# apelykh/deep-audio-mixer

Hardware: AMD Instinct MI355X
Metric: stem-spectrogram-frames/sec (train) (higher is better)
Workload: dtype f32; 1 GPU; C3: model_resnet (ResNet18, 8 stems) train step incl. STFT front-end, 8-stem 3 s @ 44.1 kHz stereo clips, n_fft 2048 hop 1024 -> 8x1025x130 per clip; batch_per_gpu=8, global_batch=8, parallelism=dp1, hip_graph=True, world_size=1, device_index=0, grad_buckets=1, allreduce_overlap=False

## Files before the change

### deep-audio-mixer_amd/_lib.py

```python
import ctypes
import os

import torch
import torch.utils.data

_HERE = os.path.dirname(os.path.abspath(__file__))
LIB_PATH = os.environ.get('DAM_LIB_PATH') or os.path.join(_HERE, 'libdam_hip.so')

EXPECTED_ABI = 26

_STATUS = {0: 'DAM_OK', -1: 'DAM_ERR_BAD_ARG', -2: 'DAM_ERR_UNSUPPORTED', -3: 'DAM_ERR_LAUNCH',
           -4: 'DAM_ERR_WORKSPACE'}

c_i, c_i64, c_f, c_p = ctypes.c_int, ctypes.c_int64, ctypes.c_float, ctypes.c_void_p
c_d = ctypes.c_double

SIGNATURES = {
    'dam_arch': (ctypes.c_char_p, []),
    'dam_abi_version': (c_i, []),
    'dam_host_dontfork_pinned': (c_i, [c_p, c_p]),
    'dam_step_mark_create': (c_i, [c_p]),
    'dam_step_mark_record': (c_i, [c_p, c_p]),
    'dam_step_mark_wait': (c_i, [c_p, c_p]),
    'dam_step_mark_synchronize': (c_i, [c_p]),
    'dam_step_mark_destroy': (c_i, [c_p]),
    'dam_stft_twiddle_count': (c_i64, [c_i]),
    'dam_stft_fill_twiddles_host': (c_i, [c_i, c_p]),
    'dam_stft_logmag_f32': (c_i, [c_p, c_i, c_i64, c_i64, c_i, c_i64, c_p, c_p, c_p, c_i, c_i, c_f, c_i, c_p, c_p]),
    'dam_stft_logmag_strided_f32': (c_i, [c_p, c_i, c_i64, c_i64, c_i64, c_i64, c_i64, c_i, c_i64, c_i64, c_p, c_p, c_p,
                                          c_i, c_i, c_f, c_i, c_p, c_p, c_i, c_p]),
    'dam_stft_complex_f32': (c_i, [c_p, c_i, c_i64, c_i64, c_i, c_i64, c_i64, c_i64, c_p, c_p, c_p, c_i, c_i, c_p, c_p]),
    'dam_stft_complex_strided_f32': (c_i, [c_p, c_i, c_i64, c_i64, c_i64, c_i64, c_i64, c_i64, c_i64, c_i, c_i64, c_i64,
                                           c_p, c_p, c_p, c_i, c_i, c_p, c_p]),
    'dam_istft_workspace_bytes': (c_i64, [c_i64, c_i64, c_i, c_i, c_i64]),
    'dam_istft_f32': (c_i, [c_p, c_p, c_i64, c_i64, c_i, c_i, c_i64, c_p, c_p, c_p, c_p, c_i64, c_p]),
    'dam_augment_gains_f32': (c_i, [ctypes.c_uint64, c_p, c_i64, c_i, c_i, c_f, c_f, c_p, c_p]),
    'dam_conv_packed_weight_count': (c_i64, [c_i, c_i, c_i, c_i]),
    'dam_conv_pack_weights_f32': (c_i, [c_p, c_i, c_i, c_i, c_i, c_i, c_p, c_p]),
    'dam_conv_pack_weights_multi_f32': (c_i, [c_p, c_i, c_i64, c_p]),
    'dam_conv2d_tapgrid_f32': (c_i, [c_p, c_i, c_i, c_i, c_i, c_i, c_p, c_i, c_i, c_p, c_p, c_p, c_i, c_i, c_p] +
                               [c_i] * 17 + [c_p, c_p, c_p, c_p, c_p, c_p, c_i64, c_p, c_p]),
    'dam_conv_batch_bytes': (c_i64, []),
    'dam_conv_batch_init': (c_i, [c_p]),
    'dam_conv_batch_flush': (c_i, [c_p, c_p]),
    'dam_conv_last_launch': (c_i, [c_p]),
    'dam_conv2d_wgrad_workspace_floats': (c_i64, [c_i, c_i, c_i, c_i]),
    'dam_conv2d_wgrad_f32': (c_i, [c_p, c_i, c_i, c_i, c_i, c_i, c_p, c_p, c_i, c_p] + [c_i] * 9 +
                             [c_p, c_i, c_p, c_i64, c_p, c_p]),
    'dam_wgrad_queue_bytes': (c_i64, []),
    'dam_wgrad_queue_init': (c_i, [c_p]),
    'dam_wgrad_queue_pending': (c_i, [c_p]),
    'dam_wgrad_queue_flush': (c_i, [c_p, c_p]),
    'dam_wgrad_queue_set_batching': (c_i, [c_p, c_i]),
    'dam_bn_workspace_floats': (c_i64, [c_i]),
    'dam_bn_stats_f32': (c_i, [c_p, c_i64, c_i, c_p, c_p, c_p, c_p, c_p, c_f, c_f, c_p, c_p, c_p, c_p, c_p, c_p]),
    'dam_bn_finalize_f32': (c_i, [c_p, c_i, c_i, c_p, c_p, c_p, c_p, c_p, c_f, c_f, c_p, c_p, c_p, c_p, c_p]),
    'dam_conv1x1_pair_f32': (c_i, [c_p, c_p, c_i, c_p, c_p, c_i, c_i, c_i, c_i, c_i, c_i, c_p, c_i, c_i, c_i, c_i, c_i, c_p]),
    'dam_dgrad_s2_3x3_f32': (c_i, [c_p, c_p, c_p, c_p, c_i, c_i, c_i, c_i, c_i, c_p, c_i, c_i, c_p, c_p, c_p, c_p]),
    'dam_conv_s2_pair_fwd_f32': (c_i, [c_p, c_p, c_p, c_i, c_i, c_i, c_i, c_i, c_p, c_p, c_p, c_p, c_p, c_p]),
    'dam_bn_finalize_pair_f32': (c_i, [c_p, c_p, c_i, c_i, c_p, c_p, c_p]),
    'dam_strip_diag_counters': (c_i, [c_p, c_i]),
    'dam_bn_stats_partial_f32': (c_i, [c_p, c_i64, c_i, c_p, c_p, c_p]),
    'dam_bn_finalize_apply_f32': (c_i, [c_p, c_i, c_i, c_p, c_p, c_i64, c_p, c_p, c_p, c_i, c_p, c_p, c_p]),
    'dam_bn_eval_affine_f32': (c_i, [c_i, c_p, c_p, c_p, c_p, c_f, c_p, c_p, c_p, c_p, c_p]),
    'dam_bn_apply_f32': (c_i, [c_p, c_i64, c_i, c_p, c_p, c_p, c_p, c_p, c_i, c_p, c_p, c_p]),
    'dam_bn_stats_pair_f32': (c_i, [c_p, c_p, c_i64, c_i, c_p, c_p, c_p, c_p]),
    'dam_bn_pair_workspace_floats': (c_i64, [c_i]),
    'dam_bn_backward_pair_f32': (c_i, [c_p, c_p, c_p, c_i64, c_i, c_i] + [c_p] * 16),
    'dam_bn_backward_f32': (c_i, [c_p, c_p, c_p, c_i64, c_i, c_p, c_p, c_p, c_i, c_p, c_p, c_p, c_p, c_p, c_p, c_p, c_i, c_p]),
    'dam_channel_sum_f32': (c_i, [c_p, c_i64, c_i, c_i, c_p, c_p, c_p]),
    'dam_dropout_tick': (c_i, [c_p, c_i64, c_p, c_p]),
    'dam_dropout_apply_f32': (c_i, [c_p, c_i64, c_f, ctypes.c_uint64, c_p, c_p, c_p]),
    'dam_heads_fwd_f32': (c_i, [c_p, c_i, c_i, c_i, c_i, c_p, c_p, c_p, c_p, c_p, c_p, c_p]),
    'dam_heads_bwd_workspace_floats': (c_i64, [c_i, c_i, c_i, c_i]),
    'dam_heads_bwd_f32': (c_i, [c_p, c_p, c_p, c_i, c_i, c_i, c_i, c_p, c_p, c_p, c_p, c_p, c_p, c_p, c_p, c_p]),
    'dam_masksum_fwd_f32': (c_i, [c_p, c_p, c_i, c_i, c_i64, c_p, c_p]),
    'dam_masksum_workspace_floats': (c_i64, [c_i, c_i]),
    'dam_masksum_bwd_f32': (c_i, [c_p, c_p, c_i, c_i, c_i64, c_p, c_p, c_p]),
    'dam_masksum_mse_f32': (c_i, [c_p, c_p, c_p, c_i, c_i, c_i64, c_p, c_p, c_p, c_p, c_p]),
    'dam_adam_l2_step_f32': (c_i, [c_p, c_p, c_p, c_p, c_i64, c_p, c_p, c_f, c_f, c_f, c_f, c_f, c_f, c_p, c_p]),
    'dam_digest64_u32': (c_i, [c_p, c_i64, c_i64, c_i, c_i, c_p, c_p]),
    'dam_gains_smooth': (c_i, [c_p, c_i, c_i, c_i, c_i, c_p, c_p, c_p, c_p]),
    'dam_gain_ramp_apply': (c_i, [c_p, c_i, c_p, c_i64, c_i64, c_i64, c_i, c_p, c_i, c_p]),
    'dam_mixdown_workspace_elems': (c_i64, [c_i64]),
    'dam_mixdown_peak_normalize': (c_i, [c_p, c_i, c_p, c_i, c_i64, c_i64, c_i, c_i, c_p, c_i, c_p, c_p]),
    'dam_nchw_to_nhwc16_f32': (c_i, [c_p, c_i, c_i, c_i64, c_p, c_p]),
    'dam_loudness_kweight_coeffs': (c_i, [c_d, c_p]),
    'dam_loudness_workspace_bytes': (c_i64, [c_i64, c_i]),
    'dam_loudness_block_energy': (c_i, [c_p, c_i, c_i64, c_i, c_i64, c_i64, c_p, c_p, c_p, c_i, c_d, c_p, c_p, c_p]),
    'dam_loudness_batch_workspace_bytes': (c_i64, [c_i, c_i64, c_i, c_i]),
    'dam_loudness_block_energy_batch': (c_i, [c_p, c_i, c_i, c_i64, c_i, c_i64, c_i64, c_i64, c_p, c_i, c_p, c_p, c_p, c_i,
                                              c_d, c_p, c_p, c_p]),
    'dam_loudness_gate': (c_i, [c_p, c_i, c_i, c_i, c_p, c_p]),
    'dam_loudness_target_gains': (c_i, [c_p, c_p, c_i, c_p, c_p]),
    'dam_pcm_tile_frames': (c_i64, [c_i]),
    'dam_pcm_max_blocks': (c_i, []),
    'dam_pcm_encode': (c_i, [c_p, c_i, c_i, c_i64, c_p, c_i, c_i, c_i, ctypes.c_uint64, c_p, c_p, c_p]),
    'dam_true_peak_taps_host': (c_i, [c_p]),
    'dam_true_peak_tile_samples': (c_i64, []),
    'dam_true_peak_max_blocks': (c_i, []),
    'dam_true_peak_workspace_bytes': (c_i64, [c_i, c_i64, c_i]),
    'dam_true_peak_batch': (c_i, [c_p, c_i, c_i, c_i64, c_i, c_i64, c_i64, c_i64, c_p, c_i, c_p, c_p, c_p, c_p]),
    'dam_peak_limit_gains': (c_i, [c_p, c_p, c_i, c_i, c_d, c_p]),
    'dam_limiter_tile_samples': (c_i64, []),
    'dam_limiter_max_lookahead': (c_i, []),
    'dam_limiter_max_hold': (c_i, []),
    'dam_limiter_workspace_bytes': (c_i64, [c_i, c_i64]),
    'dam_limiter_apply': (c_i, [c_p, c_i, c_i, c_i64, c_i, c_i64, c_i64, c_i64, c_p, c_d, c_i, c_i, c_p, c_i, c_p, c_p, c_p, c_p]),
    'dam_loudness_window_power': (c_i, [c_p, c_i, c_i, c_i, c_i, c_p, c_p, c_p]),
    'dam_loudness_curve_stats': (c_i, [c_p, c_i, c_i, c_p, c_p]),
    'dam_loudness_profile_error': (c_i, [c_p, c_p, c_i, c_i, c_i, c_p, c_p, c_p]),
    'dam_spectrum_frames_per_block': (c_i, []),
    'dam_spectrum_max_bands': (c_i, []),
    'dam_spectrum_workspace_bytes': (c_i64, [c_i, c_i64, c_i, c_i]),
    'dam_spectrum_band_power': (c_i, [c_p, c_i, c_i, c_i, c_i, c_i64, c_i64, c_i64, c_i64, c_i64, c_p, c_i, c_p, c_p, c_i, c_i,
                                      c_p, c_i, c_p, c_p, c_p]),
    'dam_spectrum_balance_error': (c_i, [c_p, c_p, c_i, c_i, c_p, c_p, c_p]),
    'dam_gainfit_tile_samples': (c_i64, []),
    'dam_gainfit_workspace_bytes': (c_i64, [c_i, c_i64, c_i]),
    'dam_gainfit_moments': (c_i, [c_p, c_i, c_i, c_i, c_i64, c_i64, c_i64, c_i64, c_p, c_i, c_i64, c_i64, c_i, c_p, c_p, c_p]),
    'dam_gainfit_solve': (c_i, [c_p, c_i, c_i, c_i, c_d, c_p, c_p, c_p, c_p]),
    'dam_gainfit_gain_error': (c_i, [c_p, c_p, c_i, c_i, c_i, c_i, c_p, c_p, c_p, c_p]),
}
# ... 59 lines not shown
```

### deep-audio-mixer_amd/csrc/dam_conv.hip

```cpp
#include <cstdlib>
#include "dam_common.h"
#include "dam_conv_geo.h"
#include "dam_conv_stage.h"

namespace dam {

namespace {

typedef float v4f __attribute__((ext_vector_type(4)));

constexpr int GEO_PACK_MAX = 4;
struct ConvGeoPack {
    ConvGeo g[GEO_PACK_MAX];
    int n, B;
};

template <int MB, int NB>
__global__ __launch_bounds__(256) void conv_igemm_kernel(const ConvGeoPack pk, const float* __restrict__ X,
                                                         const float4* __restrict__ Wp, const float* __restrict__ bias,
                                                         const float* __restrict__ in_scale,
                                                         const float* __restrict__ in_shift, float* __restrict__ Y,
                                                         const float* __restrict__ res, const float* __restrict__ res_mask,
                                                         float* __restrict__ splitk_ws) {
    extern __shared__ __attribute__((aligned(16))) unsigned char smem[];
// ... 431 lines not shown
        DAM_PAIR_MFMA(xa, wa)
        DAM_PAIR_MFMA(xb, wb)
    } else {
        float4 xa[R], wa[R][NB], xb[R], wb[R][NB];
        const int rounds = (nch + R - 1) / R, total = 2 * rounds;
        DAM_PAIR_LOAD(xr1, wr1, tap1, 0, xa, wa)
#pragma unroll 1
        for (int r = 0; r < total; r += 2) {
            {
                const int q = r + 1, c0 = (q >= rounds ? q - rounds : q) * R;
                if (q >= rounds) { DAM_PAIR_LOAD(xr2, wr2, tap2, c0, xb, wb) } else { DAM_PAIR_LOAD(xr1, wr1, tap1, c0, xb, wb) }
            }
            DAM_PAIR_MFMA(xa, wa)
            if (r + 2 < total) {
                const int q = r + 2, c0 = (q >= rounds ? q - rounds : q) * R;
                if (q >= rounds) { DAM_PAIR_LOAD(xr2, wr2, tap2, c0, xa, wa) } else { DAM_PAIR_LOAD(xr1, wr1, tap1, c0, xa, wa) }
            }
            DAM_PAIR_MFMA(xb, wb)
        }
    }
#undef DAM_PAIR_LOAD
#undef DAM_PAIR_MFMA
    if (!valid) return;
    const size_t opix = ((size_t)img * OHt + (oh * os + oo_h)) * OWt + (ow * os + oo_w);
#pragma unroll
    for (int nb = 0; nb < NB; ++nb) {
        const int ch = (nb0 + nb) * 16 + kq * 4;
        *reinterpret_cast<float4*>(Y + opix * N + ch) = make_float4(acc[nb].x, acc[nb].y, acc[nb].z, acc[nb].w);
    }
}

template <int NB, int NCHMAX>
int launch_conv1x1(const ConvGeo& g, const float* X, const float* Wp, const float* bias, float* Y, const float* res,
                   const float* res_mask, hipStream_t st) {
    const int segs = (int)cdiv(g.Wo, 16);
    const int64_t units = (int64_t)g.B * g.Ho * segs;
    if (units >= (1ll << 30)) return DAM_ERR_UNSUPPORTED;
    hipLaunchKernelGGL((conv1x1_direct_kernel<NB, NCHMAX>), dim3((unsigned)cdiv(units, 4), (unsigned)(g.N / 16 / NB)), dim3(256), 0, st,
                       g, X, reinterpret_cast<const float4*>(Wp), bias, Y, res, res_mask, segs, (int)units);
    DAM_CHECK_LAUNCH();
    conv_last_launch = ConvLaunchNote{CONV_FAM_1X1, 0, NB, NCHMAX, 0, 0, 0, 0, 0, 0, 0, 1, 1};
    return DAM_OK;
}

}
}

extern "C" int dam_conv1x1_pair_f32(const float* x1, const float* w1_packed, int tap1, const float* x2, const float* w2_packed,
                                    int tap2, int B, int H, int W, int C, int n_out, float* y, int OHt, int OWt, int out_stride,
                                    int out_off_h, int out_off_w, void* stream) {
    using namespace dam;
    if (!x1 || !w1_packed || !x2 || !w2_packed || !y || B <= 0 || H <= 0 || W <= 0 || tap1 < 0 || tap2 < 0 || out_stride < 1)
        return DAM_ERR_BAD_ARG;
    if (C % 16 || n_out % 16 || C <= 0 || n_out <= 0) return DAM_ERR_UNSUPPORTED;
    if ((H - 1) * out_stride + out_off_h >= OHt || (W - 1) * out_stride + out_off_w >= OWt || out_off_h < 0 || out_off_w < 0)
        return DAM_ERR_BAD_ARG;
    if ((int64_t)B * H * W * C * 4 >= (1ll << 31)) return DAM_ERR_UNSUPPORTED;
    const int segs = (int)cdiv(W, 16);
    const int64_t units = (int64_t)B * H * segs;
    if (units >= (1ll << 30)) return DAM_ERR_UNSUPPORTED;
    const int nblk = n_out / 16, nch = C / 16;
    hipStream_t st = (hipStream_t)stream;
#define DAM_PAIR_GO(NB_, R_, BOTH_)                                                                                           \
    hipLaunchKernelGGL((conv1x1_pair_kernel<NB_, R_, BOTH_>), dim3((unsigned)cdiv(units, 4), (unsigned)(nblk / NB_)), dim3(256), 0, st, x1, \
                       reinterpret_cast<const float4*>(w1_packed), tap1, x2, reinterpret_cast<const float4*>(w2_packed), tap2, B, H, W, \
                       C, n_out, y, OHt, OWt, out_stride, out_off_h, out_off_w, segs, (int)units)
    if (nblk % 2 == 0) {
        if (nch <= 2) DAM_PAIR_GO(2, 2, true); else if (nch <= 4) DAM_PAIR_GO(2, 4, true); else DAM_PAIR_GO(2, 4, false);
    } else {
        if (nch <= 2) DAM_PAIR_GO(1, 2, true); else if (nch <= 4) DAM_PAIR_GO(1, 4, true); else DAM_PAIR_GO(1, 8, false);
    }
#undef DAM_PAIR_GO
    DAM_CHECK_LAUNCH();
    return DAM_OK;
}

namespace dam {
thread_local ConvLaunchNote conv_last_launch{};
}

extern "C" int dam_conv_last_launch(int* out16_host) {
    if (!out16_host) return DAM_ERR_BAD_ARG;
    const dam::ConvLaunchNote& n = dam::conv_last_launch;
    const int v[16] = {n.family, n.MB, n.NB, n.NCH, n.T33, n.LW, n.EPI, n.SO, n.PU, n.STATS, n.KS, n.ksplit, n.ranges, 0, 0, 0};
    for (int i = 0; i < 16; ++i) out16_host[i] = v[i];
    return DAM_OK;
}

extern "C" int64_t dam_conv_batch_bytes(void) { return (int64_t)sizeof(dam::ConvBatch); }

extern "C" int dam_conv_batch_init(void* batch) {
    if (!batch) return DAM_ERR_BAD_ARG;
    dam::ConvBatch* b = static_cast<dam::ConvBatch*>(batch);
    b->magic = dam::CONV_BATCH_MAGIC;
    b->n = 0;
    return DAM_OK;
}

extern "C" int dam_conv_batch_flush(void* batch, void* stream) {
    dam::ConvBatch* b = static_cast<dam::ConvBatch*>(batch);
    if (!b || b->magic != dam::CONV_BATCH_MAGIC) return DAM_ERR_BAD_ARG;
    return dam::conv_batch_flush(*b, (hipStream_t)stream);
}

extern "C" int dam_conv2d_tapgrid_f32(const float* x, int B, int H, int W, int C, int in_nchw, const float* w_packed,
                                      int k_chunks, int n_out, const float* bias, const float* in_scale,
                                      const float* in_shift, int relu_in, int relu_out, float* y, int OHt, int OWt, int Ho, int Wo,
                                      int out_stride, int out_off_h, int out_off_w, int in_stride, int nA, int nB,
                                      int off_h, int step_h, int off_w, int step_w, int wt_base, int wt_sa, int wt_sb,
                                      const float* res, const float* res_mask, float* bn_partial, int* bn_parts_host,
                                      const dam_bn_bwd_sums* bn_bwd, float* workspace, int64_t workspace_floats,
                                      void* batch, void* stream) {
    using namespace dam;
    conv_last_launch = ConvLaunchNote{};
    if (bn_parts_host) *bn_parts_host = 0;
    BnBwdEpi bwd{};
    if (bn_bwd && bn_bwd->x) {
        if (!bn_partial || !bn_parts_host || !bn_bwd->mean || !bn_bwd->invstd) return DAM_ERR_BAD_ARG;
        if (bn_bwd->mask_bits ? (bn_bwd->mask_scale || bn_bwd->mask_shift || !res) : (!bn_bwd->mask_scale || !bn_bwd->mask_shift))
            return DAM_ERR_BAD_ARG;
        if (res && (!bn_bwd->res_mask_bits || !res_mask)) return DAM_ERR_BAD_ARG;
        bwd = BnBwdEpi{bn_bwd->x, bn_bwd->mean, bn_bwd->invstd, bn_bwd->mask_scale, bn_bwd->mask_shift, bn_bwd->res_mask_bits,
                       bn_bwd->mask_bits};
    }
    if (!x || !w_packed || !y || B <= 0 || H <= 0 || W <= 0 || C <= 0 || Ho <= 0 || Wo <= 0 || nA <= 0 || nB <= 0)
        return DAM_ERR_BAD_ARG;
    if (n_out % 16 || (in_stride != 1 && in_stride != 2) || out_stride < 1) return DAM_ERR_UNSUPPORTED;
    if (in_nchw ? (C > 16 || k_chunks != 1) : (C % 16 || k_chunks != C / 16)) return DAM_ERR_UNSUPPORTED;
    if (in_scale && !in_shift) return DAM_ERR_BAD_ARG;
    if (B > 65535) return DAM_ERR_UNSUPPORTED;
    ConvGeo g;
    g.B = B; g.H = H; g.W = W; g.C = C; g.Ho = Ho; g.Wo = Wo; g.N = n_out; g.OHt = OHt; g.OWt = OWt;
    g.os = out_stride; g.oo_h = out_off_h; g.oo_w = out_off_w; g.s = in_stride; g.nA = nA; g.nB = nB;
    g.off_h = off_h; g.step_h = step_h; g.off_w = off_w; g.step_w = step_w;
    g.wt_base = wt_base; g.wt_sa = wt_sa; g.wt_sb = wt_sb;
    g.in_nchw = in_nchw; g.relu_in = relu_in; g.relu_out = relu_out != 0; g.nchunks = k_chunks; g.NBtot = n_out / 16;
    g.epi_bwd = 0;
    const int h_lo = off_h + (step_h < 0 ? (nA - 1) * step_h : 0), h_hi = off_h + (step_h > 0 ? (nA - 1) * step_h : 0);
    const int w_lo = off_w + (step_w < 0 ? (nB - 1) * step_w : 0), w_hi = off_w + (step_w > 0 ? (nB - 1) * step_w : 0);
    g.r0 = h_lo; g.c0 = w_lo;
    g.PWin = (Wo - 1) * in_stride + (w_hi - w_lo) + 1;
    g.PWs = (int)cdiv(g.PWin, in_stride);
    g.PWT = g.PWs * in_stride;

    hipStream_t st = (hipStream_t)stream;
    g.PR = 0; g.CG = 1; g.tiles_m = 0; g.ksplit = 1; g.gps = 1 << 30;
    if (nA == 1 && nB == 1 && !in_nchw && !in_scale && k_chunks <= 8 &&
        (int64_t)B * H * W * C * 4 < (1ll << 31) && (int64_t)B * OHt * OWt * n_out * 4 < (1ll << 62)) {
        const int nblk = n_out / 16;
        if (k_chunks <= 2) return nblk % 2 == 0 ? launch_conv1x1<2, 2>(g, x, w_packed, bias, y, res, res_mask, st)
                                                : launch_conv1x1<1, 2>(g, x, w_packed, bias, y, res, res_mask, st);
        if (k_chunks <= 4) return nblk % 2 == 0 ? launch_conv1x1<2, 4>(g, x, w_packed, bias, y, res, res_mask, st)
                                                : launch_conv1x1<1, 4>(g, x, w_packed, bias, y, res, res_mask, st);
        return nblk % 2 == 0 ? launch_conv1x1<2, 8>(g, x, w_packed, bias, y, res, res_mask, st)
                             : launch_conv1x1<1, 8>(g, x, w_packed, bias, y, res, res_mask, st);
    }
    if (!in_nchw) {
        int parts = 0;
        const int rc = conv_strip_try(g, h_lo, h_hi, x, w_packed, bias, y, res, res_mask, bn_partial, &parts,
                                      in_scale, in_shift, bwd, st);
        if (rc == DAM_OK) {
            if (bn_partial && bn_parts_host) *bn_parts_host = parts;
            return DAM_OK;
        }
        if (rc != DAM_ERR_UNSUPPORTED) return rc;
        if (bn_partial) {
            const int rc2 = conv_strip_try(g, h_lo, h_hi, x, w_packed, bias, y, res, res_mask, nullptr, nullptr, in_scale, in_shift,
                                           BnBwdEpi{}, st);
            if (rc2 == DAM_OK) return DAM_OK;
            if (rc2 != DAM_ERR_UNSUPPORTED) return rc2;
        }
    }
    if (!getenv("DAM_NO_PIPE")) {
        int parts = 0;
        const int rc = conv_pipe_try(g, h_hi - h_lo, x, w_packed, bias, in_scale, in_shift, y, res, res_mask, workspace,
                                     (bwd.x && res) ? nullptr : bn_partial, &parts, (bwd.x && res) ? BnBwdEpi{} : bwd, st);
        if (rc == DAM_OK && bn_partial && bn_parts_host) *bn_parts_host = parts;
        if (rc != DAM_ERR_UNSUPPORTED) return rc;
        if (nA == 3 && nB == 3 && !in_nchw && !bn_partial) {
            for (int ns = 2; ns <= 4; ++ns) {
                const int wd0 = (int)cdiv(Wo, ns);
                if (wd0 < 16) break;
                int rc2 = DAM_OK, done = 0;
                for (int ow0 = 0; ow0 < Wo && rc2 == DAM_OK; ow0 += wd0, ++done) {
                    ConvGeo g2 = g;
                    g2.Wo = Wo - ow0 < wd0 ? Wo - ow0 : wd0;
                    g2.oo_w = out_off_w + ow0 * out_stride;
                    g2.off_w = off_w + ow0 * in_stride;
                    g2.c0 = w_lo + ow0 * in_stride;
                    g2.PWin = (g2.Wo - 1) * in_stride + (w_hi - w_lo) + 1;
                    g2.PWs = (int)cdiv(g2.PWin, in_stride);
                    g2.PWT = g2.PWs * in_stride;
                    rc2 = conv_pipe_try(g2, h_hi - h_lo, x, w_packed, bias, in_scale, in_shift, y, res, res_mask, workspace, nullptr,
                                        nullptr, BnBwdEpi{}, st);
                }
                if (rc2 == DAM_OK) {
                    conv_last_launch.family = CONV_FAM_PIPE_RANGES;
                    conv_last_launch.ranges = done;
                    return DAM_OK;
                }
                if (rc2 != DAM_ERR_UNSUPPORTED || done > 1) return rc2 == DAM_ERR_UNSUPPORTED ? DAM_ERR_LAUNCH : rc2;
            }
        }
    }
    const int64_t npix = (int64_t)Ho * Wo;
    const int nblk = n_out / 16;
    int MB = 4, NB = nblk % 4 == 0 ? 4 : (nblk % 3 == 0 ? 3 : (nblk % 2 == 0 ? 2 : 1));
    auto wgs = [&](int mb, int nb) { return cdiv(npix, 64 * mb) * cdiv(nblk, nb) * B; };
    const bool can_split = workspace && out_stride == 1 && Ho == OHt && Wo == OWt && out_off_h == 0 && out_off_w == 0 &&
                           k_chunks >= 4;
    bool split = can_split;
    if (split) {
        int64_t best = -1;
        for (int mb = 4; mb >= 1; mb >>= 1) {
            const int64_t w = wgs(mb, NB);
            if (w < 400) continue;
            const int64_t cost = cdiv(w, 256) * (mb * NB + 1);
            if (best < 0 || cost < best) { best = cost; MB = mb; split = false; }
        }
    }
// ... 67 lines not shown
```

### deep-audio-mixer_amd/csrc/dam_conv_geo.h

```cpp
#pragma once
#include "dam_common.h"

namespace dam {

struct ConvGeo {
    int B, H, W, C;
    int Ho, Wo;
    int N;
    int OHt, OWt;
    int os, oo_h, oo_w;
    int s;
    int nA, nB;
    int off_h, step_h, off_w, step_w;
    int wt_base, wt_sa, wt_sb;
    int r0, c0;
    int PR, PWin, PWs, PWT;
    int nchunks, CG;
    int NBtot;
    int tiles_m;
    int in_nchw;
    int relu_in;
    int relu_out;
    int ksplit;
    int gps;
    int epi_bwd;
};

struct BnBwdEpi {
    const float* x;
    const float* mean; const float* invstd; const float* mscale; const float* mshift;
    const unsigned char* res_bits;
    const unsigned char* mask_bits;
};

struct StripGeo {
    int NR;
    int RH;
    int tiles_m, tpw, strips;
    int ring_off;
    int w_lds;
    int w_taps;
    unsigned wo_magic;
};

enum ConvFamily { CONV_FAM_NONE = 0, CONV_FAM_STRIP = 1, CONV_FAM_PIPE = 2, CONV_FAM_PIPE_RANGES = 3, CONV_FAM_TILE = 4,
                  CONV_FAM_TILE_BATCH = 5, CONV_FAM_1X1 = 6 };
struct ConvLaunchNote {
    int family, MB, NB, NCH, T33, LW, EPI, SO, PU, STATS, KS, ksplit, ranges;
};
extern thread_local ConvLaunchNote conv_last_launch;

int conv_strip_try(ConvGeo& g, int h_lo, int h_hi, const float* X, const float* Wp, const float* bias, float* Y,
                   const float* res, const float* res_mask, float* stats, int* stats_parts,
                   const float* in_scale, const float* in_shift, const BnBwdEpi& bwd, hipStream_t st);

int conv_pipe_try(ConvGeo g, int row_span, const float* X, const float* Wp, const float* bias, const float* sc, const float* sh,
                  float* Y, const float* res, const float* res_mask, float* workspace, float* stats, int* stats_parts,
                  const BnBwdEpi& bwd, hipStream_t st);

}
```

### deep-audio-mixer_amd/csrc/dam_conv_strip.hip

```cpp
#include <algorithm>
#include <cstdint>
#include "dam_common.h"
#include "dam_conv_geo.h"

namespace dam {
namespace {

typedef float v4f __attribute__((ext_vector_type(4)));
typedef int v4i __attribute__((ext_vector_type(4)));
typedef float v2f __attribute__((ext_vector_type(2)));

#ifdef DAM_STRIP_DIAG_TAGS
}
__device__ unsigned strip_diag_counters[2];
namespace {
#endif

#ifdef DAM_STAMPS
#define DAM_STAMP(slot)                                                                                   \
    do {                                                                                                  \
        if (lane == 0 && (wave == 0 || wave == NCW) && stamp_i < 30)                                        \
            reinterpret_cast<unsigned long long*>(stats)[(((size_t)blockIdx.z * gridDim.x + blockIdx.x) * 2 + (wave == NCW)) * 32 + \
                                                         (stamp_i++)] = __builtin_amdgcn_s_memtime() | ((unsigned long long)(slot) << 56); \
    } while (0)
#else
#define DAM_STAMP(slot) do { } while (0)
#endif

__device__ __forceinline__ int fdiv(int e, int d, float inv_d) {
    int q = (int)((float)e * inv_d);
    if (q * d > e) --q;
    if ((q + 1) * d <= e) ++q;
    return q;
}

constexpr int STRIP_LOADERS = 4;
constexpr int STRIP_THREADS = 512 + 64 * STRIP_LOADERS;
constexpr int STRIP_PU = 8;

struct RowLoad {
    const float* ximg;
    int H, W, C, s, c0, PWs, PWin, PWT, nchunks, RB, CHB, NR, ring_off, ppr, gpp;
    float inv_ppr, inv_gpp;
    int m_ppr, m_gpp;
};

__device__ __forceinline__ void rows_issue(const RowLoad& r, int lo, int hi, int first, int part, int nparts, int lane,
                                           float4 (&lv)[STRIP_PU], int (&ldst)[STRIP_PU], int (&laff)[STRIP_PU]) {
    const int total = (hi - lo + 1) * r.ppr;
#pragma unroll
    for (int u = 0; u < STRIP_PU; ++u) {
        const int q = first + part + nparts * u;
        const bool used = q < total;
        const int qc = used ? q : total - 1;
        const int row = (qc * r.m_ppr) >> 16, rem = qc - row * r.ppr;
        const int cc = (rem * r.m_gpp) >> 16, gi = rem - cc * r.gpp;
        const int ih = lo + row;
        const int L = gi * 64 + lane, slot = L >> 2, quad = L & 3;
        int pw = slot;
        if (r.s != 1) pw = slot < r.PWs ? 2 * slot : 2 * (slot - r.PWs) + 1;
        const int iw = pw + r.c0;
        const bool col_ok = slot < r.PWT && pw < r.PWin && iw >= 0 && iw < r.W;
        const bool inb = used && col_ok && ih >= 0 && ih < r.H;
        const int ihc = ih < 0 ? 0 : (ih >= r.H ? r.H - 1 : ih), iwc = iw < 0 ? 0 : (iw >= r.W ? r.W - 1 : iw);
        const float4 x = *reinterpret_cast<const float4*>(r.ximg + (unsigned)((ihc * r.W + iwc) * r.C + cc * 16 + quad * 4));
        lv[u] = inb ? x : make_float4(0.f, 0.f, 0.f, 0.f);
        ldst[u] = (used && col_ok) ? cc * r.CHB + ((ih + r.ring_off) & (r.NR - 1)) * r.RB + L * 16 : -1;
        laff[u] = inb ? cc : -1;
    }
}
template <int NCH>
__device__ __forceinline__ float4 in_affine(float4 v, int cc, const v4f (&scq)[NCH], const v4f (&shq)[NCH], bool relu) {
    const v4f sc = (NCH > 1 && cc > 0) ? scq[NCH - 1] : scq[0], sh = (NCH > 1 && cc > 0) ? shq[NCH - 1] : shq[0];
    float4 o = make_float4(fmaf(v.x, sc.x, sh.x), fmaf(v.y, sc.y, sh.y), fmaf(v.z, sc.z, sh.z), fmaf(v.w, sc.w, sh.w));
    if (relu) { o.x = fmaxf(o.x, 0.f); o.y = fmaxf(o.y, 0.f); o.z = fmaxf(o.z, 0.f); o.w = fmaxf(o.w, 0.f); }
    return o;
}
template <int NCH>
__device__ __forceinline__ void rows_commit(unsigned char* smem, const float4 (&lv)[STRIP_PU], int (&ldst)[STRIP_PU],
                                            const int (&laff)[STRIP_PU], bool has_aff, const v4f (&scq)[NCH],
                                            const v4f (&shq)[NCH], bool relu) {
#pragma unroll
    for (int u = 0; u < STRIP_PU; ++u) {
        if (ldst[u] >= 0) {
            float4 v = lv[u];
            if (has_aff && laff[u] >= 0) v = in_affine<NCH>(v, laff[u], scq, shq, relu);
            *reinterpret_cast<float4*>(smem + ldst[u]) = v;
        }
        ldst[u] = -1;
    }
}

template <int MB, int NB, int NCH, bool T33, bool LW, int EPI, int SO>
__global__ __launch_bounds__(SO ? 512 : STRIP_THREADS, 1) void conv_strip_kernel(const ConvGeo g, const StripGeo sg, const float* __restrict__ X,
                                                         const float4* __restrict__ Wp, const float* __restrict__ bias,
                                                         float* __restrict__ Y, const float* __restrict__ res,
                                                         const float* __restrict__ res_mask, float* __restrict__ stats,
                                                         const float* __restrict__ in_scale, const float* __restrict__ in_shift,
                                                         const BnBwdEpi bwd) {
    extern __shared__ __attribute__((aligned(16))) unsigned char smem[];
    const int tid = threadIdx.x, lane = tid & 63;
    const int wave = __builtin_amdgcn_readfirstlane(tid >> 6);
    const int j = lane & 15, kq = lane >> 4;
    constexpr int MW = 16 * MB, TM = 4 * MW;
    constexpr int NT = SO ? 512 : STRIP_THREADS;
    constexpr int NCW = SO ? 4 : 8, LGRP = SO ? 1 : 2;
    const int img = blockIdx.z, nb0 = blockIdx.y * NB;
    const int HoWo = g.Ho * g.Wo;
    const int t_begin = blockIdx.x * sg.tpw;
    int t_end = t_begin + sg.tpw;
    if (t_end > sg.tiles_m) t_end = sg.tiles_m;
    const int RB = g.PWT * 64;
    const int CHB = sg.NR * RB;
    const int RH = sg.RH;
    const float* ximg = X + (size_t)img * g.H * g.W * g.C;
    const bool has_aff = in_scale != nullptr, relu_in = g.relu_in != 0, relu_out = g.relu_out != 0;
    v4f scq[NCH], shq[NCH];
#pragma unroll
    for (int c = 0; c < NCH; ++c) {
        scq[c] = has_aff ? *reinterpret_cast<const v4f*>(in_scale + c * 16 + (lane & 3) * 4) : (v4f){1.f, 1.f, 1.f, 1.f};
        shq[c] = has_aff ? *reinterpret_cast<const v4f*>(in_shift + c * 16 + (lane & 3) * 4) : (v4f){0.f, 0.f, 0.f, 0.f};
    }
#ifdef DAM_STAMPS
    int stamp_i = 0;
#endif
    DAM_STAMP(1);


    auto tile_rows = [&](int t, int& lo, int& hi) {
        const int p0 = t * TM;
        int p1 = p0 + TM - 1;
        if (p1 > HoWo - 1) p1 = HoWo - 1;
        lo = (int)__umulhi((unsigned)p0, sg.wo_magic) * g.s + g.r0;
        hi = (int)__umulhi((unsigned)p1, sg.wo_magic) * g.s + g.r0 + RH - 1;
    };
    const int groups_per_plane = (g.PWT * 4 + 63) >> 6;
    const int pieces_per_row = g.nchunks * groups_per_plane;
    const float inv_ppr = 1.0f / (float)pieces_per_row, inv_gpp = 1.0f / (float)groups_per_plane;
    float4 lv[STRIP_PU];
    int ldst[STRIP_PU], laff[STRIP_PU];
#pragma unroll
    for (int u = 0; u < STRIP_PU; ++u) ldst[u] = -1;
    RowLoad rl;
    rl.ximg = ximg; rl.H = g.H; rl.W = g.W; rl.C = g.C; rl.s = g.s; rl.c0 = g.c0; rl.PWs = g.PWs; rl.PWin = g.PWin; rl.PWT = g.PWT;
    rl.nchunks = g.nchunks; rl.RB = RB; rl.CHB = CHB; rl.NR = sg.NR; rl.ring_off = sg.ring_off;
    rl.ppr = pieces_per_row; rl.gpp = groups_per_plane; rl.inv_ppr = inv_ppr; rl.inv_gpp = inv_gpp;
    rl.m_ppr = (int)(65536.0f * inv_ppr) + 1; rl.m_gpp = (int)(65536.0f * inv_gpp) + 1;

    const int grp = wave >> 2, cw = wave & 3;
    const int n_tiles = t_end - t_begin;
    const int n_slots = (n_tiles + 2) & ~1;
    int lo0, hi0;
    tile_rows(t_begin, lo0, hi0);
    constexpr int HS = (NCH == 1 && !LW && SO != 0) ? 2 : 1;
    constexpr int KP = (NCH == 1 ? 1 : (LW ? 2 : 3)) * HS;
    constexpr int GPPF = NCH == 1 ? (LW ? 14 : 9) : (LW ? 7 : 5);
    constexpr int GPP = (GPPF + HS - 1) / HS;
    const int hsel = HS == 2 ? (wave & 1) : 0;
    int loffb[GPP];
    unsigned long long cmask[GPP];
#pragma unroll
    for (int gu = 0; gu < GPP; ++gu) {
        const int gi = gu * HS + hsel;
        const int L = gi * 64 + lane, slot = L >> 2, quad = L & 3;
        int pw = slot;
        if (g.s != 1) pw = slot < g.PWs ? 2 * slot : 2 * (slot - g.PWs) + 1;
        const int iw = pw + g.c0;
        const bool ok = gi < groups_per_plane && slot < g.PWT && pw < g.PWin && iw >= 0 && iw < g.W;
        const int iwc = iw < 0 ? 0 : (iw >= g.W ? g.W - 1 : iw);
        loffb[gu] = (iwc * g.C + quad * 4) * 4;
        cmask[gu] = __ballot(ok);
    }
    const __amdgpu_buffer_rsrc_t xrsrc = __builtin_amdgcn_make_buffer_rsrc(const_cast<float*>(ximg), 0, g.H * g.W * g.C * 4, 0x00020000);
    const int lane16 = lane * 16 + hsel * 1024;
    const v4f zero4 = {0.f, 0.f, 0.f, 0.f};
    const float relu_lo = relu_in ? 0.f : -__builtin_inff();
// ... 401 lines not shown
                if (nvalid <= 0) continue;
                const int oh_m = (int)__umulhi((unsigned)pm, sg.wo_magic), ow_m = pm - oh_m * g.Wo;
                const int voff = __builtin_amdgcn_readfirstlane(oh_m * oA + ow_m * oB) + (lane_o + wflag[mb] * oD);
                if (j < nvalid) {
#pragma unroll
                    for (int nb = 0; nb < NB; ++nb) {
                        v4f v = acc[mb][nb] + bias4[nb];
                        if (res) {
                            v4f rv, mv;
                            if constexpr (EPI >= 2) { rv = res_pf[mb][nb]; }
                            else if constexpr (RES_PF) { rv = res_pf[mb][nb]; mv = msk_pf[mb][nb]; }
                            else {
                                rv = __builtin_bit_cast(v4f, __builtin_amdgcn_raw_buffer_load_b128(rrsrc, voff + nb * 64, 0, 0));
                                if (res_mask) mv = __builtin_bit_cast(v4f, __builtin_amdgcn_raw_buffer_load_b128(mrsrc, voff + nb * 64, 0, 0));
                            }
                            if constexpr (EPI >= 2) {
                                const int b8 = mskb_pf[mb][nb];
                                v.x += (b8 & 1) ? rv.x : 0.f; v.y += (b8 & 2) ? rv.y : 0.f;
                                v.z += (b8 & 4) ? rv.z : 0.f; v.w += (b8 & 8) ? rv.w : 0.f;
                            } else if constexpr (EPI == 1) {
                                const v4f m = __builtin_elementwise_fma(rv, bw_ms[nb], bw_mh[nb]);
                                const v4f xh = __builtin_elementwise_fma(rv, bw_k1[nb], bw_k2[nb]);
                                v4f dz;
                                dz.x = m.x > 0.f ? v.x : 0.f; dz.y = m.y > 0.f ? v.y : 0.f;
                                dz.z = m.z > 0.f ? v.z : 0.f; dz.w = m.w > 0.f ? v.w : 0.f;
                                st_s1[nb][0] += dz.xy; st_s1[nb][1] += dz.zw;
                                st_s2[nb][0] = __builtin_elementwise_fma(dz.xy, xh.xy, st_s2[nb][0]);
                                st_s2[nb][1] = __builtin_elementwise_fma(dz.zw, xh.zw, st_s2[nb][1]);
                            } else if (res_mask) {
                                v.x += mv.x > 0.f ? rv.x : 0.f; v.y += mv.y > 0.f ? rv.y : 0.f;
                                v.z += mv.z > 0.f ? rv.z : 0.f; v.w += mv.w > 0.f ? rv.w : 0.f;
                            } else {
                                v += rv;
                            }
                        }
                        if (relu_out) v = __builtin_elementwise_max(v, (v4f){0.f, 0.f, 0.f, 0.f});
                        __builtin_amdgcn_raw_buffer_store_b128(__builtin_bit_cast(v4i, v), yrsrc, voff + nb * 64, 0, 0);
                        if constexpr (EPI >= 2) {
                            const v4f xq = x_pf[mb][nb];
                            const v4f xh = __builtin_elementwise_fma(xq, bw_k1[nb], bw_k2[nb]);
                            v4f dz;
                            if constexpr (EPI == 3) {
                                const int ub = upb_pf[mb][nb];
                                dz.x = (ub & 1) ? v.x : 0.f; dz.y = (ub & 2) ? v.y : 0.f;
                                dz.z = (ub & 4) ? v.z : 0.f; dz.w = (ub & 8) ? v.w : 0.f;
                            } else {
                                const v4f m = __builtin_elementwise_fma(xq, bw_ms[nb], bw_mh[nb]);
                                dz.x = m.x > 0.f ? v.x : 0.f; dz.y = m.y > 0.f ? v.y : 0.f;
                                dz.z = m.z > 0.f ? v.z : 0.f; dz.w = m.w > 0.f ? v.w : 0.f;
                            }
                            st_s1[nb][0] += dz.xy; st_s1[nb][1] += dz.zw;
                            st_s2[nb][0] = __builtin_elementwise_fma(dz.xy, xh.xy, st_s2[nb][0]);
                            st_s2[nb][1] = __builtin_elementwise_fma(dz.zw, xh.zw, st_s2[nb][1]);
                        }
#ifndef DAM_STAMPS
                        if (stats && !epi_bwd) {
                            if (!st_have) { st_nk[nb][0] = -v.xy; st_nk[nb][1] = -v.zw; }
                            const v2f d0 = v.xy + st_nk[nb][0], d1 = v.zw + st_nk[nb][1];
                            st_s1[nb][0] += d0; st_s1[nb][1] += d1;
                            st_s2[nb][0] = __builtin_elementwise_fma(d0, d0, st_s2[nb][0]);
                            st_s2[nb][1] = __builtin_elementwise_fma(d1, d1, st_s2[nb][1]);
                        }
#endif
                    }
                    if (stats) ++st_n;
                }
                st_have = true;
            }
            }
            if constexpr (T33) {
                if (s + 1 < n_tiles) DAM_STRIP_GEOM(s + 1);
            }
            DAM_STAMP(6);
        }
        asm volatile("s_waitcnt lgkmcnt(0)\n\ts_barrier" ::: "memory");
        DAM_STAMP(7);
    }

    if constexpr (SO != 0) {
        static_assert(T33, "the self-overlapped form is built on the compile-time 3x3 item grid");
        if (grp == 0) {
            constexpr bool ST = EPI == 0 && SO == 2, BIAS = EPI == 0 && (SO == 3 || SO == 4), RADD = EPI == 0 && SO == 4,
                           RMSK = EPI == 0 && SO == 5, NEED_R = EPI != 0 || RADD || RMSK;
            constexpr int NI = 9 * NCH;
            static_assert(NI >= 2 * MB + 1, "one filler per item: MB write-out units, MB geometry units, the operand prefetch");
            v4f accX[2][MB][NB];
            int voffX[2][MB];
            int baseX[2][3][MB];
            v4f rpf[NEED_R ? MB : 1][NEED_R ? NB : 1], mpf[RMSK ? MB : 1][RMSK ? NB : 1], xpf[EPI >= 2 ? MB : 1][EPI >= 2 ? NB : 1];
            int mbpf[EPI >= 2 ? MB : 1][EPI >= 2 ? NB : 1], ubpf[EPI == 3 ? MB : 1][EPI == 3 ? NB : 1];
            const float floor_out = relu_out ? 0.f : -3.0e38f;
            const int lane_oD = lane_o + oD;
            float4 wa[2][NB], xv[2][MB];

            v4i tq[MB][2];
#ifdef DAM_STRIP_DIAG_TAGS
            int tq_want[MB];
#define SO_TAG_EXPECT(T_, MBI_) tq_want[MBI_] = SO_TAG(T_)
#define SO_TAG_CHECK(QA_, MBI_)                                                                                           \
    do {                                                                                                                  \
        if (lane == 0) {                                                                                                  \
            atomicAdd(&strip_diag_counters[0], 1u);                                                                       \
            if (((QA_).y & 0x7fff0000) != tq_want[MBI_]) atomicAdd(&strip_diag_counters[1], 1u);                          \
        }                                                                                                                 \
        (QA_).y &= 0xffff;                                                                                                \
    } while (0)
#else
#define SO_TAG_EXPECT(T_, MBI_) do { } while (0)
#define SO_TAG_CHECK(QA_, MBI_) do { } while (0)
#endif
#define SO_TABREAD(T_, MBI_)                                                                                              \
    do {                                                                                                                  \
        const int ta_ = tab_base + ((cw * 4 + ((T_) & 3)) * MB + (MBI_)) * 32;                                            \
        tq[MBI_][0] = *reinterpret_cast<const v4i*>(smem + ta_);                                                          \
        tq[MBI_][1] = *reinterpret_cast<const v4i*>(smem + ta_ + 16);                                                     \
        SO_TAG_EXPECT(T_, MBI_);                                                                                          \
    } while (0)
#define SO_GEOM(P_, MBI_)                                                                                                 \
    do {                                                                                                                  \
        v4i qa_ = tq[MBI_][0];                                                                                            \
        const v4i qb_ = tq[MBI_][1];                                                                                      \
        SO_TAG_CHECK(qa_, MBI_);                                                                                          \
        const bool nx_ = j >= qa_.y;                                                                                      \
        voffX[P_][MBI_] = (nx_ ? lane_oD : lane_o) + qa_.x;                                                               \
        baseX[P_][0][MBI_] = lane_x + (nx_ ? qb_.y : qa_.z);                                                              \
        baseX[P_][1][MBI_] = lane_x + (nx_ ? qb_.z : qa_.w);                                                              \
        baseX[P_][2][MBI_] = lane_x + (nx_ ? qb_.w : qb_.x);                                                              \
    } while (0)
#define SO_LOAD(P_, I_, BUF_)                                                                                             \
    do {                                                                                                                  \
        constexpr int a_ = (I_) / (3 * NCH), b_ = ((I_) / NCH) % 3, cc_ = (I_) % NCH;                                     \
        _Pragma("unroll") for (int nb = 0; nb < NB; ++nb)                                                                 \
            wa[BUF_][nb] = *reinterpret_cast<const float4*>(smem + w_lane + ((((a_ * 3 + b_) * NCH + cc_) * NB + nb) * 1024)); \
        _Pragma("unroll") for (int mb = 0; mb < MB; ++mb)                                                                 \
            xv[BUF_][mb] = *reinterpret_cast<const float4*>(smem + (cc_ ? baseX[P_][a_][mb] + CHB : baseX[P_][a_][mb]) + b_ * 64); \
    } while (0)
#define SO_MFMA(P_, I_, BUF_)                                                                                             \
    do {                                                                                                                  \
        _Pragma("unroll") for (int r = 0; r < 4; ++r)                                                                     \
            _Pragma("unroll") for (int mb = 0; mb < MB; ++mb)                                                             \
                _Pragma("unroll") for (int nb = 0; nb < NB; ++nb)                                                         \
                    accX[P_][mb][nb] = __builtin_amdgcn_mfma_f32_16x16x4f32(                                              \
                        reinterpret_cast<const float*>(&wa[BUF_][nb])[r], reinterpret_cast<const float*>(&xv[BUF_][mb])[r], \
                        ((I_) == 0 && r == 0) ? (v4f){0.f, 0.f, 0.f, 0.f} : accX[P_][mb][nb], 0, 0, 0);                   \
    } while (0)
#define SO_PREFETCH1(P_, MBI_)                                                                                            \
    do {                                                                                                                  \
        if constexpr (NEED_R) {                                                                                           \
            const int vo_ = voffX[P_][MBI_];                                                                              \
            _Pragma("unroll") for (int nb = 0; nb < NB; ++nb) {         \
                rpf[MBI_][nb] = __builtin_bit_cast(v4f, __builtin_amdgcn_raw_buffer_load_b128(rrsrc, vo_ + nb * 64, 0, 0)); \
                if constexpr (RMSK)                                                                                       \
                    mpf[MBI_][nb] = __builtin_bit_cast(v4f, __builtin_amdgcn_raw_buffer_load_b128(mrsrc, vo_ + nb * 64, 0, 0)); \
                if constexpr (EPI >= 2) {                                                                                 \
                    mbpf[MBI_][nb] = (int)__builtin_amdgcn_raw_buffer_load_b8(bbrsrc, (vo_ >> 4) + nb * 4, 0, 0);         \
                    xpf[MBI_][nb] = __builtin_bit_cast(v4f, __builtin_amdgcn_raw_buffer_load_b128(x2rsrc, vo_ + nb * 64, 0, 0)); \
                }                                                                                                         \
                if constexpr (EPI == 3)                                                                                   \
                    ubpf[MBI_][nb] = (int)__builtin_amdgcn_raw_buffer_load_b8(ubrsrc, (vo_ >> 4) + nb * 4, 0, 0);         \
            }                                                                                                             \
        }                                                                                                                 \
    } while (0)
#define SO_UNIT(Q_, T_, MBI_, PRED_)                                                                                      \
    do {                                                                                                                  \
             \
          \
                                    \
        const int vo_ = voffX[Q_][MBI_];                                                                                  \
        if (!(PRED_) || j < HoWo - ((t_begin + (T_)) * TM + cw * MW + (MBI_) * 16)) {                                     \
            _Pragma("unroll") for (int nb = 0; nb < NB; ++nb) {                                                           \
                v4f v = accX[Q_][MBI_][nb];                                                                               \
                if constexpr (BIAS) {                                                                                     \
                    v += bias4[nb];                                                                                       \
                    if constexpr (RADD) v += rpf[MBI_][nb];                                                               \
                    v.x = fmaxf(v.x, floor_out); v.y = fmaxf(v.y, floor_out); v.z = fmaxf(v.z, floor_out); v.w = fmaxf(v.w, floor_out); \
                }                                                                                                         \
                if constexpr (RMSK) {                                                                                     \
                    const v4f rv = rpf[MBI_][nb], mv = mpf[MBI_][nb];                                                     \
                    v.x += mv.x > 0.f ? rv.x : 0.f; v.y += mv.y > 0.f ? rv.y : 0.f;                                       \
                    v.z += mv.z > 0.f ? rv.z : 0.f; v.w += mv.w > 0.f ? rv.w : 0.f;                                       \
                }                                                                                                         \
                if constexpr (EPI >= 2) {              \
                    const v4f rv = rpf[MBI_][nb];                                                                         \
                    const int b8 = mbpf[MBI_][nb];                                                                        \
                    v.x += (b8 & 1) ? rv.x : 0.f; v.y += (b8 & 2) ? rv.y : 0.f;                                           \
                    v.z += (b8 & 4) ? rv.z : 0.f; v.w += (b8 & 8) ? rv.w : 0.f;                                           \
                }                                                                                                         \
                __builtin_amdgcn_raw_buffer_store_b128(__builtin_bit_cast(v4i, v), yrsrc, vo_ + nb * 64, 0, 0);           \
                if constexpr (EPI != 0) {            \
                    const v4f xq = EPI == 1 ? rpf[MBI_][nb] : xpf[MBI_][nb];                                              \
                    const v4f xh = __builtin_elementwise_fma(xq, bw_k1[nb], bw_k2[nb]);                                   \
                    v4f dz;                                                                                               \
                    if constexpr (EPI == 3) {                                                                             \
                        const int ub = ubpf[MBI_][nb];                                                                    \
                        dz.x = (ub & 1) ? v.x : 0.f; dz.y = (ub & 2) ? v.y : 0.f;                                         \
                        dz.z = (ub & 4) ? v.z : 0.f; dz.w = (ub & 8) ? v.w : 0.f;                                         \
                    } else {                                                                                              \
                        const v4f m = __builtin_elementwise_fma(xq, bw_ms[nb], bw_mh[nb]);                                \
                        dz.x = m.x > 0.f ? v.x : 0.f; dz.y = m.y > 0.f ? v.y : 0.f;                                       \
                        dz.z = m.z > 0.f ? v.z : 0.f; dz.w = m.w > 0.f ? v.w : 0.f;                                       \
                    }                                                                                                     \
                    st_s1[nb][0] += dz.xy; st_s1[nb][1] += dz.zw;                                                         \
                    st_s2[nb][0] = __builtin_elementwise_fma(dz.xy, xh.xy, st_s2[nb][0]);                                 \
                    st_s2[nb][1] = __builtin_elementwise_fma(dz.zw, xh.zw, st_s2[nb][1]);                                 \
                }                                                                                                         \
                if constexpr (ST) {                                                                                       \
                    const v2f d0 = v.xy + st_nk[nb][0], d1 = v.zw + st_nk[nb][1];                                         \
                    st_s1[nb][0] += d0; st_s1[nb][1] += d1;                                                               \
                    st_s2[nb][0] = __builtin_elementwise_fma(d0, d0, st_s2[nb][0]);                                       \
                    st_s2[nb][1] = __builtin_elementwise_fma(d1, d1, st_s2[nb][1]);                                       \
                }                                                                                                         \
            }                                                                                                             \
            if constexpr (ST) ++st_n;                                                                                     \
        }                                                                                                                 \
    } while (0)
#define SO_FILL(P_, S_, I_, WO_)                                                                                          \
    do {                                                                                                                  \
          \
         \
        int sa_ = (S_);                                                                                                   \
        asm volatile("" : "+s"(sa_));                                                                                     \
        if constexpr ((I_) < MB) {                                                                                        \
            if constexpr (WO_) SO_UNIT(1 - (P_), sa_ - 1, ((I_) < MB ? (I_) : 0), 0);                                     \
            SO_TABREAD(sa_ + 1, ((I_) < MB ? (I_) : 0));                                                                  \
            SO_PREFETCH1(P_, ((I_) < MB ? (I_) : 0));                                                                     \
        } else if constexpr ((I_) < 2 * MB) SO_GEOM(1 - (P_), ((I_) < 2 * MB && (I_) >= MB ? (I_) - MB : 0));             \
    } while (0)
#define SO_PATTERN()                                                                                                      \
    do {                                                                                                                  \
        _Pragma("unroll") for (int q_ = 0; q_ < 4 * MB * NB; ++q_) {                                                      \
            __builtin_amdgcn_sched_group_barrier(0x008, 1, 0);                                                            \
            __builtin_amdgcn_sched_group_barrier(0x100, 1, 0);                                                            \
            __builtin_amdgcn_sched_group_barrier(0x002, 3, 0);                                                            \
            __builtin_amdgcn_sched_group_barrier(0x004, 2, 0);                                                            \
            __builtin_amdgcn_sched_group_barrier(0x030, 1, 0);                                                            \
        }                                                                                                                 \
    } while (0)
#define SO_ITEM(P_, S_, I_, WO_)                                                                                          \
    do {                                                                                                                  \
        if constexpr ((I_) + 1 < NI) SO_LOAD(P_, ((I_) + 1 < NI ? (I_) + 1 : 0), ((I_) + 1) & 1);                         \
        SO_MFMA(P_, I_, (I_) & 1);                                                                                        \
        if constexpr ((I_) != 0) SO_FILL(P_, S_, I_, WO_);                                                                \
        SO_PATTERN();                                                                                                     \
        __builtin_amdgcn_sched_barrier(0);                                                                                \
    } while (0)
#define SO_SLOT(P_, S_, WO_)                                                                                              \
    do {                                                                                                                  \
          \
                       \
        SO_LOAD(P_, 0, 0);                                                                                                \
        SO_FILL(P_, S_, 0, WO_);                                                                                          \
        __builtin_amdgcn_sched_barrier(0);                                                                                \
        SO_ITEM(P_, S_, 0, WO_); SO_ITEM(P_, S_, 1, WO_); SO_ITEM(P_, S_, 2, WO_); SO_ITEM(P_, S_, 3, WO_); SO_ITEM(P_, S_, 4, WO_); \
        SO_ITEM(P_, S_, 5, WO_); SO_ITEM(P_, S_, 6, WO_); SO_ITEM(P_, S_, 7, WO_); SO_ITEM(P_, S_, 8, WO_);               \
        if constexpr (NCH == 2) {                                                                                         \
            SO_ITEM(P_, S_, 9, WO_); SO_ITEM(P_, S_, 10, WO_); SO_ITEM(P_, S_, 11, WO_); SO_ITEM(P_, S_, 12, WO_); SO_ITEM(P_, S_, 13, WO_); \
            SO_ITEM(P_, S_, 14, WO_); SO_ITEM(P_, S_, 15, WO_); SO_ITEM(P_, S_, 16, WO_); SO_ITEM(P_, S_, 17, WO_);       \
        }                                                                                                                 \
        DAM_STAMP(5);                                                                                                     \
        asm volatile("s_waitcnt lgkmcnt(0)\n\ts_barrier" ::: "memory");                                                   \
        DAM_STAMP(7);                                                                                                     \
    } while (0)
#define SO_LAST(Q_, T_)                                                                                                   \
    do {                                                                                                                  \
         \
           \
         \
        asm volatile("s_nop 15\n\ts_nop 15" ::: "memory");                                                                \
        _Pragma("unroll") for (int mb = 0; mb < MB; ++mb) {                                                               \
            if (HoWo - ((t_begin + (T_)) * TM + cw * MW + mb * 16) > 0) SO_UNIT(Q_, T_, mb, 1);                           \
        }                                                                                                                 \
        asm volatile("s_waitcnt lgkmcnt(0)\n\ts_barrier" ::: "memory");                                                   \
        DAM_STAMP(7);                                                                                                     \
    } while (0)

#pragma unroll
            for (int mb = 0; mb < MB; ++mb) { SO_TABREAD(0, mb); SO_GEOM(0, mb); }
            SO_SLOT(0, 0, 0);
            if constexpr (ST) {
                asm volatile("s_nop 15\n\ts_nop 15" ::: "memory");
#pragma unroll
                for (int nb = 0; nb < NB; ++nb) { st_nk[nb][0] = -accX[0][0][nb].xy; st_nk[nb][1] = -accX[0][0][nb].zw; }
            }
            int s = 1;
            for (; s + 1 < n_tiles; s += 2) {
                SO_SLOT(1, s, 1);
                SO_SLOT(0, s + 1, 1);
            }
            if (s < n_tiles) {
                SO_SLOT(1, s, 1);
                ++s;
            }
            if ((n_tiles - 1) & 1) SO_LAST(1, n_tiles - 1);
            else SO_LAST(0, n_tiles - 1);
            for (++s; s < n_slots; ++s) {
                asm volatile("s_waitcnt lgkmcnt(0)\n\ts_barrier" ::: "memory");
                DAM_STAMP(7);
            }
#undef SO_GEOM
#undef SO_TABREAD
#undef SO_TAG_EXPECT
#undef SO_TAG_CHECK
#undef SO_LOAD
#undef SO_MFMA
#undef SO_PREFETCH1
#undef SO_UNIT
#undef SO_FILL
#undef SO_PATTERN
#undef SO_ITEM
#undef SO_SLOT
#undef SO_LAST
        }
    }

#undef SO_TABLE
#undef SO_TAG
#undef DAM_STRIP_GEOM
#ifdef DAM_STAMPS
    DAM_STAMP(8);
    return;
#endif
    if constexpr (epi_bwd) {
        __syncthreads();
        float* sm = reinterpret_cast<float*>(smem);
#pragma unroll
        for (int nb = 0; nb < NB; ++nb)
#pragma unroll
            for (int r = 0; r < 4; ++r) {
                float a = st_s1[nb][r >> 1][r & 1], b = st_s2[nb][r >> 1][r & 1];
#pragma unroll
                for (int off = 1; off < 16; off <<= 1) { a += __shfl_xor(a, off); b += __shfl_xor(b, off); }
                if (j == 0 && wave < NCW) {
                    float* o = sm + ((wave * NB * 16) + nb * 16 + kq * 4 + r) * 2;
                    o[0] = a; o[1] = b;
                }
            }
        __syncthreads();
        if (tid < NB * 16) {
            float a = 0.f, b = 0.f;
            for (int w = 0; w < NCW; ++w) { a += sm[((w * NB * 16) + tid) * 2]; b += sm[((w * NB * 16) + tid) * 2 + 1]; }
            const int ch = nb0 * 16 + tid;
            if (ch < g.N) {
                const size_t part = (size_t)blockIdx.z * gridDim.x + blockIdx.x;
                store_sc1(stats + (part * g.N + ch) * 2, a);
                store_sc1(stats + (part * g.N + ch) * 2 + 1, b);
            }
        }
        return;
    }
    if (stats) {
        float* sm = reinterpret_cast<float*>(smem);
#pragma unroll
        for (int nb = 0; nb < NB; ++nb)
#pragma unroll
            for (int r = 0; r < 4; ++r) {
                float n = (float)st_n;
                const float s1 = st_s1[nb][r >> 1][r & 1], s2 = st_s2[nb][r >> 1][r & 1];
                const float md = st_n ? s1 / n : 0.f;
                float mean = md - st_nk[nb][r >> 1][r & 1];
                float m2 = st_n ? fmaxf(s2 - s1 * md, 0.f) : 0.f;
#pragma unroll
                for (int off = 1; off < 16; off <<= 1) {
                    const float nb_ = __shfl_xor(n, off), mb_ = __shfl_xor(mean, off), qb_ = __shfl_xor(m2, off);
                    const float nn = n + nb_;
                    if (nn > 0.f) {
                        const float d = mb_ - mean;
                        mean += d * (nb_ / nn);
                        m2 += qb_ + d * d * (n * nb_ / nn);
                    }
                    n = nn;
                }
                if (j == 0 && wave < NCW) {
                    float* o = sm + ((wave * NB * 16) + nb * 16 + kq * 4 + r) * 3;
                    o[0] = n; o[1] = mean; o[2] = m2;
                }
            }
        __syncthreads();
        if (tid < NB * 16) {
            float n = 0.f, mean = 0.f, m2 = 0.f;
            for (int w = 0; w < NCW; ++w) {
                const float* o = sm + ((w * NB * 16) + tid) * 3;
                const float nb_ = o[0];
                if (nb_ == 0.f) continue;
                const float nn = n + nb_, d = o[1] - mean;
                mean += d * (nb_ / nn);
                m2 += o[2] + d * d * (n * nb_ / nn);
                n = nn;
            }
            const int ch = nb0 * 16 + tid;
            if (ch < g.N) {
                const size_t part = (size_t)blockIdx.z * gridDim.x + blockIdx.x;
                float* o = stats + (part * g.N + ch) * 3;
                store_sc1(o, n); store_sc1(o + 1, mean); store_sc1(o + 2, m2);
            }
        }
    }
}

}

template <int MB, int NB, int NCH, bool T33, bool LW = false, int EPI = 0, int SO = 0>
static int launch_strip(ConvGeo& g, StripGeo& sg, size_t lds, const float* X, const float* Wp, const float* bias, float* Y,
                        const float* res, const float* res_mask, float* stats, const float* in_scale, const float* in_shift,
                        const BnBwdEpi& bwd, hipStream_t st) {
    if (lds > 64 * 1024 && !raise_lds_limit<&conv_strip_kernel<MB, NB, NCH, T33, LW, EPI, SO>>(160 * 1024)) return DAM_ERR_LAUNCH;
    dim3 grid((unsigned)sg.strips, (unsigned)cdiv(g.N / 16, NB), (unsigned)g.B);
    hipLaunchKernelGGL((conv_strip_kernel<MB, NB, NCH, T33, LW, EPI, SO>), grid, dim3(SO ? 512 : STRIP_THREADS), lds, st, g, sg, X, reinterpret_cast<const float4*>(Wp), bias,
                       Y, res, res_mask, stats, in_scale, in_shift, bwd);
    DAM_CHECK_LAUNCH();
    conv_last_launch = ConvLaunchNote{CONV_FAM_STRIP, MB, NB, NCH, T33, LW, EPI, SO, 0, 0, 0, 1, 1};
    return DAM_OK;
}

int conv_strip_try(ConvGeo& g_in, int h_lo, int h_hi, const float* X, const float* Wp, const float* bias, float* Y,
                   const float* res, const float* res_mask, float* stats, int* stats_parts,
                   const float* in_scale, const float* in_shift, const BnBwdEpi& bwd, hipStream_t st) {
    if (bwd.x && !stats) return DAM_ERR_BAD_ARG;
    if (bwd.x && res && !bwd.res_bits) return DAM_ERR_UNSUPPORTED;
    ConvGeo g = g_in;
    g.epi_bwd = bwd.x ? (res ? (bwd.mask_bits ? 3 : 2) : 1) : 0;
    if (bwd.x && bwd.mask_bits && !res) return DAM_ERR_UNSUPPORTED;
    if (g.nB == 3 && g.step_w < 0) {
        g.off_w += 2 * g.step_w; g.step_w = -g.step_w;
        g.wt_base += 2 * g.wt_sb; g.wt_sb = -g.wt_sb;
    }
    if (g.in_nchw || g.B > 65535 || g.nA > 3 || g.nB > 3 || g.nchunks > 2) return DAM_ERR_UNSUPPORTED;
    const int nblk = g.N / 16;
    const int64_t npix = (int64_t)g.Ho * g.Wo;
    if (npix >= (1 << 22)) return DAM_ERR_UNSUPPORTED;
    const int NB = nblk % 2 == 0 ? 2 : 1;
    if (stats && cdiv(nblk, NB) != 1) return DAM_ERR_UNSUPPORTED;
    StripGeo sg;
    sg.RH = h_hi - h_lo + 1;
    sg.w_taps = 9;
    const size_t w_bytes = (size_t)9 * g.nchunks * NB * 1024;
    if (w_bytes > 48 * 1024) return DAM_ERR_UNSUPPORTED;
    sg.w_lds = 1;
    const size_t LDS_MAX = 150 * 1024;
    int MB = 4;
    size_t lds = 0;
    bool wide = false;
    for (;; MB >>= 1) {
        const int tm = 64 * MB;
        int rows_out = (int)((tm + g.Wo - 2) / g.Wo + 1);
        if (rows_out > g.Ho) rows_out = g.Ho;
        const int rows_tile = (rows_out - 1) * g.s + sg.RH;
        const int rows_new = rows_out * g.s;
        int nr = 1;
        while (nr < rows_tile + rows_new) nr <<= 1;
        const int gpp = (g.PWT * 4 + 63) / 64;
        wide = gpp > (g.nchunks == 1 ? 9 : 5);
        const int kp = g.nchunks == 1 ? 1 : (wide ? 2 : 3), gpp_max = g.nchunks == 1 ? (wide ? 14 : 9) : (wide ? 7 : 5);
        if (gpp > gpp_max) return DAM_ERR_UNSUPPORTED;
        if (wide && MB != (g.nchunks == 1 ? 4 : 2)) { if (MB == 2) return DAM_ERR_UNSUPPORTED; continue; }
        if (rows_new * g.nchunks > STRIP_LOADERS * kp) { if (MB == 2) return DAM_ERR_UNSUPPORTED; continue; }
        lds = (size_t)nr * g.PWT * 64 * g.nchunks + w_bytes;
        if (lds <= LDS_MAX) { sg.NR = nr; break; }
        if (MB == 2) return DAM_ERR_UNSUPPORTED;
    }
    const int tm = 64 * MB;
    sg.tiles_m = (int)cdiv(npix, tm);
    int tpw = sg.tiles_m;
    int64_t slots = 256;
    {
        const int64_t per_image = cdiv(nblk, NB);
        int64_t best = INT64_MAX;
        for (int strips = 1; strips <= sg.tiles_m; ++strips) {
            const int t = (int)cdiv(sg.tiles_m, strips);
            if (t < 2 && sg.tiles_m >= 2) break;
            const int64_t wgs = (int64_t)cdiv(sg.tiles_m, t) * g.B * per_image;
            const int64_t cost = cdiv(wgs, slots) * (t + 2);
            if (cost < best) { best = cost; tpw = t; }
        }
    }
    sg.tpw = tpw;
    sg.strips = (int)cdiv(sg.tiles_m, tpw);
    if (g.Wo > 1024 || g.Wo < 16) return DAM_ERR_UNSUPPORTED;
    sg.wo_magic = (unsigned)((1ull << 32) / (unsigned)g.Wo) + 1u;
    sg.ring_off = sg.NR * 64;
    if (stats_parts) *stats_parts = sg.strips * g.B;
    if (stats && (int64_t)sg.strips * g.B > 1024) return DAM_ERR_UNSUPPORTED;
    if (lds < (size_t)8 * NB * 16 * 3 * sizeof(float)) lds = (size_t)8 * NB * 16 * 3 * sizeof(float);
    const bool t33 = g.nA == 3 && g.nB == 3 && g.s == 1 && g.step_w == 1;
#define DAM_STRIP_ARGS g, sg, lds, X, Wp, bias, Y, (bwd.x && !res ? bwd.x : res), (bwd.x && res ? reinterpret_cast<const float*>(bwd.res_bits) : res_mask), stats, in_scale, in_shift, bwd, st
    const int rows_out_so = std::min(g.Ho, (64 * MB + g.Wo - 2) / g.Wo + 1), rows_tile_so = (rows_out_so - 1) * g.s + sg.RH;
    if (t33 && !wide && rows_tile_so * g.nchunks <= 8 * (g.nchunks == 1 ? 1 : 2) &&
        ((g.nchunks == 1 && MB == 4 && NB == 1) || (g.nchunks == 2 && MB == 2 && NB == 2))) {
        const bool c16 = g.nchunks == 1;
        lds += 2048;
#define DAM_SO_CASE(E_, S_)                                                                                              \
    return c16 ? launch_strip<4, 1, 1, true, false, E_, S_>(DAM_STRIP_ARGS) : launch_strip<2, 2, 2, true, false, E_, S_>(DAM_STRIP_ARGS)
        if (bwd.x && res) {
            if (c16) {
                if (bwd.mask_bits) return launch_strip<4, 1, 1, true, false, 3, 1>(DAM_STRIP_ARGS);
                return launch_strip<4, 1, 1, true, false, 2, 1>(DAM_STRIP_ARGS);
            }
        } else if (bwd.x) {
            DAM_SO_CASE(1, 1);
        } else if (stats) {
            if (!bias && !res && !g.relu_out) DAM_SO_CASE(0, 2);
        } else if (res && res_mask) {
            if (!bias && !g.relu_out) DAM_SO_CASE(0, 5);
        } else if (res) {
            DAM_SO_CASE(0, 4);
        } else if (bias || g.relu_out) {
            DAM_SO_CASE(0, 3);
        } else {
            DAM_SO_CASE(0, 1);
        }
#undef DAM_SO_CASE
    }
    if (bwd.x && res) {
        if (!t33 || g.nchunks != 1 || MB != 4 || NB != 1) return DAM_ERR_UNSUPPORTED;
        if (bwd.mask_bits)
            return wide ? launch_strip<4, 1, 1, true, true, 3>(DAM_STRIP_ARGS) : launch_strip<4, 1, 1, true, false, 3>(DAM_STRIP_ARGS);
        return wide ? launch_strip<4, 1, 1, true, true, 2>(DAM_STRIP_ARGS) : launch_strip<4, 1, 1, true, false, 2>(DAM_STRIP_ARGS);
    }
    if (bwd.x) {
        if (!t33) return DAM_ERR_UNSUPPORTED;
        if (g.nchunks == 1 && MB == 4 && NB == 1)
            return wide ? launch_strip<4, 1, 1, true, true, 1>(DAM_STRIP_ARGS) : launch_strip<4, 1, 1, true, false, 1>(DAM_STRIP_ARGS);
        if (g.nchunks == 2 && MB == 2 && NB == 2)
            return wide ? launch_strip<2, 2, 2, true, true, 1>(DAM_STRIP_ARGS) : launch_strip<2, 2, 2, true, false, 1>(DAM_STRIP_ARGS);
        return DAM_ERR_UNSUPPORTED;
    }
#define DAM_STRIP_CASE(M_, N_)                                                                                           \
    if (MB == M_ && NB == N_) {                                                                                             \
        if (t33) return g.nchunks == 1 ? launch_strip<M_, N_, 1, true>(DAM_STRIP_ARGS) : launch_strip<M_, N_, 2, true>(DAM_STRIP_ARGS); \
        return g.nchunks == 1 ? launch_strip<M_, N_, 1, false>(DAM_STRIP_ARGS) : launch_strip<M_, N_, 2, false>(DAM_STRIP_ARGS); \
    }
    if (wide) {
        if (g.nchunks == 1 && MB == 4 && NB == 1)
            return t33 ? launch_strip<4, 1, 1, true, true>(DAM_STRIP_ARGS) : launch_strip<4, 1, 1, false, true>(DAM_STRIP_ARGS);
        if (g.nchunks == 2 && MB == 2 && NB == 2)
            return t33 ? launch_strip<2, 2, 2, true, true>(DAM_STRIP_ARGS) : launch_strip<2, 2, 2, false, true>(DAM_STRIP_ARGS);
        return DAM_ERR_UNSUPPORTED;
    }
    DAM_STRIP_CASE(4, 2); DAM_STRIP_CASE(4, 1);
    DAM_STRIP_CASE(2, 2); DAM_STRIP_CASE(2, 1);
#undef DAM_STRIP_CASE
#undef DAM_STRIP_ARGS
    return DAM_ERR_UNSUPPORTED;
}

}

extern "C" int dam_strip_diag_counters(uint32_t* out2_host, int reset) {
#ifdef DAM_STRIP_DIAG_TAGS
    if (!out2_host) return DAM_ERR_BAD_ARG;
    if (hipDeviceSynchronize() != hipSuccess) return DAM_ERR_LAUNCH;
    unsigned v[2] = {0, 0};
    if (hipMemcpyFromSymbol(v, HIP_SYMBOL(dam::strip_diag_counters), sizeof(v)) != hipSuccess) return DAM_ERR_LAUNCH;
    out2_host[0] = v[0]; out2_host[1] = v[1];
    if (reset) {
        const unsigned z[2] = {0, 0};
        if (hipMemcpyToSymbol(HIP_SYMBOL(dam::strip_diag_counters), z, sizeof(z)) != hipSuccess) return DAM_ERR_LAUNCH;
    }
    return DAM_OK;
#else
    (void)out2_host; (void)reset;
    return DAM_ERR_UNSUPPORTED;
#endif
}
```

### deep-audio-mixer_amd/csrc/dam_wgrad.hip

```cpp
#include <string.h>
#include "dam_common.h"
#include "dam_conv_stage.h"

namespace dam {

struct WgradGeo {
    int B, H, W, C;
    int Ho, Wo, N;
    int s;
    int KH, KW;
    int off_h, step_h, off_w, step_w;
    int r0, c0;
    int PR, PWin, PWs, PWT;
    int nchunks;
    int nblk;
    int tiles_n, tiles_k, tap_groups;
    int tiles_m, total_tiles, nsplit;
    int in_nchw, relu_in;
    int TMW;
};

constexpr int WG_MAX_JOBS = 4;
struct WgradJobs {
    const float* X[WG_MAX_JOBS];
// ... 246 lines not shown
    WgradJobs jobs;
    float* dw[WG_MAX_JOBS];
    int64_t ws_floats[WG_MAX_JOBS];
    int n_real[WG_MAX_JOBS], k_real[WG_MAX_JOBS];
    int (*launch)(WgradQueue*, hipStream_t);
};
struct PendingDirect {
    int sig;
    DirectJobs jobs;
    float* dw[WD_MAX_JOBS];
    int n_real[WD_MAX_JOBS], k_real[WD_MAX_JOBS];
    int (*launch)(WgradQueue*, hipStream_t);
};
struct WgradQueue {
    unsigned magic;
    int batching;
    ReduceBatch batch;
    PendingTile pend;
    PendingDirect pend_direct;
};
constexpr unsigned WGRAD_QUEUE_MAGIC = 0x57475251u;

int reduce_flush(ReduceBatch& b, hipStream_t st) {
    if (b.njobs <= 0) return DAM_OK;
    int blocks = 0;
    for (int i = 0; i < b.njobs; ++i) blocks += b.job[i].blocks;
    hipLaunchKernelGGL(wgrad_reduce_batch_kernel, dim3(blocks), dim3(256), 0, st, b);
    b.njobs = 0;
    DAM_CHECK_LAUNCH();
    return DAM_OK;
}

int reduce_submit(void* queue, const float* partial, float* dw, int nsplit, int nx, int TNB, int TKB, int TA, int TB, int n_real,
                  int k_real, int KH, int KW, int tap_groups, int tiles_k, hipStream_t st) {
    ReduceJob j;
    j.partial = partial; j.dw = dw; j.nsplit = nsplit; j.nx = nx; j.TNB = TNB; j.TKB = TKB; j.TA = TA; j.TB = TB;
    j.n_real = n_real; j.k_real = k_real; j.KH = KH; j.KW = KW; j.tap_groups = tap_groups; j.tiles_k = tiles_k;
    const int64_t per_split4 = (int64_t)nx * TNB * TKB * TA * TB * 64;
    if (nsplit >= 64) {
        j.sl = 32;
        j.blocks = (int)(cdiv(per_split4, 8) < 4096 ? cdiv(per_split4, 8) : 4096);
    } else if (per_split4 >= 8192) {
        j.sl = 1;
        j.blocks = (int)(cdiv(per_split4, 256) < 4096 ? cdiv(per_split4, 256) : 4096);
    } else {
        j.sl = 8;
        j.blocks = (int)(cdiv(per_split4, 32) < 2048 ? cdiv(per_split4, 32) : 2048);
    }
    if (!queue) {
        ReduceBatch one;
        one.job[0] = j; one.njobs = 1;
        return reduce_flush(one, st);
    }
    WgradQueue* q = static_cast<WgradQueue*>(queue);
    if (q->magic != WGRAD_QUEUE_MAGIC) return DAM_ERR_BAD_ARG;
    if (q->batch.njobs == REDUCE_MAX_JOBS) {
        const int rc = reduce_flush(q->batch, st);
        if (rc != DAM_OK) return rc;
    }
    q->batch.job[q->batch.njobs++] = j;
    return DAM_OK;
}

struct RowsGeo {
    int B, H, W, C;
    int P4;
    int rps, spi;
    int tiles_k;
    int gpp;
};
#ifdef DAM_WGR_STAMPS
#define DAM_WSTAMP(tag)                                                                                                \
    do {                                                                                                              \
        if (lane == 0 && (wave == 0 || wave == 4) && stamp_n < 32)                                                    \
            stamp_v[stamp_n++] = ((unsigned long long)(tag) << 56) | ((unsigned long long)__builtin_readcyclecounter() & ((1ull << 56) - 1)); \
    } while (0)
#else
#define DAM_WSTAMP(tag) do { } while (0)
#endif
constexpr int RW_LOADERS = 8;
constexpr int RW_THREADS = 256 + 64 * RW_LOADERS, RW_GUARD = 64, RW_TAIL = 1280;
template <int D> __device__ __forceinline__ int rw_mod(int v) { return D == 10 ? v - ((v * 52429) >> 19) * 10 : v - ((v * 43691) >> 18) * 6; }

template <int TNB, int TKB, int STEPS, int KP, int GPP, int HV, int NL>
__global__ __launch_bounds__(256 + 64 * NL) void wgrad_rows_kernel(const RowsGeo g, const float* __restrict__ X,
                                                                const float* __restrict__ dY, const float* __restrict__ in_scale,
                                                                const float* __restrict__ in_shift, int relu_in,
                                                                float* __restrict__ partial) {
    extern __shared__ __attribute__((aligned(16))) unsigned char smem[];
    constexpr int NBLK = TNB * TKB * 9;
    constexpr int RPS = 4 / HV, RW_NRX = 2 * RPS + 2, RW_NRD = 2 * RPS;
    const int tid = threadIdx.x, lane = tid & 63;
    const int wave = __builtin_amdgcn_readfirstlane(tid >> 6);
    const int j = lane & 15, kq = lane >> 4;
    int bx = blockIdx.x, by = blockIdx.y;
    {
        const int nxg = gridDim.x, L = blockIdx.y * nxg + blockIdx.x, full = (gridDim.y >> 3) << 3;
        if (L < full * nxg) { const int c = L & 7, r = L >> 3; bx = r % nxg; by = (r / nxg) * 8 + c; }
    }
    const int tn = bx / g.tiles_k, tk = bx - tn * g.tiles_k;
    const int img = by / g.spi, sidx = by - img * g.spi;
    const int r_begin = (int)(((long long)sidx * g.H) / g.spi), r_end = (int)(((long long)(sidx + 1) * g.H) / g.spi);
    const int n_slots = (r_end - r_begin + RPS - 1) / RPS;
    const int n_slots2 = (n_slots + 1) & ~1;
    const int ROWB = g.P4 * 64;
    const int XPLANE = RW_NRX * ROWB, DPLANE = RW_NRD * ROWB;
    const int XBASE = RW_GUARD, DBASE = XBASE + TKB * XPLANE;
    const int lds_bytes = DBASE + TNB * DPLANE + RW_TAIL;

#define DAM_RW_ZERO()                                                                                                      \
    do {                                                                                                                   \
        const int npad_ = g.P4 - g.W, nrow_ = TKB * RW_NRX + TNB * RW_NRD;                                                 \
        for (int e = tid; e < nrow_ * npad_ * 4; e += (256 + 64 * NL)) {                                                        \
            const int q_ = e & 3, c_ = (e >> 2) % npad_, r_ = (e >> 2) / npad_;                                            \
            const int cell_ = c_ == 0 ? 0 : g.W + c_;                                                                      \
            *reinterpret_cast<float4*>(smem + XBASE + r_ * ROWB + cell_ * 64 + q_ * 16) = make_float4(0.f, 0.f, 0.f, 0.f); \
        }                                                                                                                  \
        for (int e = tid * 16; e < RW_GUARD; e += (256 + 64 * NL) * 16)                                                         \
            *reinterpret_cast<float4*>(smem + e) = make_float4(0.f, 0.f, 0.f, 0.f);                                        \
        for (int e = tid * 16; e < RW_TAIL; e += (256 + 64 * NL) * 16)                                                          \
            *reinterpret_cast<float4*>(smem + lds_bytes - RW_TAIL + e) = make_float4(0.f, 0.f, 0.f, 0.f);                  \
    } while (0)

    v4f acc[NBLK];
#pragma unroll
    for (int i = 0; i < NBLK; ++i) acc[i] = (v4f){0.f, 0.f, 0.f, 0.f};
#ifdef DAM_WGR_STAMPS
    unsigned long long stamp_v[32];
    int stamp_n = 0;
#pragma unroll
    for (int i = 0; i < 32; ++i) stamp_v[i] = 0;
#endif
    DAM_WSTAMP(1);

    if (wave >= 4) {
        const int cwl = wave - 4;
        int loffb[GPP];
        unsigned long long cmask[GPP];
#pragma unroll
        for (int gi = 0; gi < GPP; ++gi) {
            const int L = gi * 64 + lane, e = L >> 2, quad = L & 3, col = e - 1;
            const bool ok = gi < g.gpp && e < g.P4 && col >= 0 && col < g.W;
            const int colc = col < 0 ? 0 : (col >= g.W ? g.W - 1 : col);
            loffb[gi] = (colc * g.C + quad * 4) * 4;
            cmask[gi] = __ballot(ok);
        }
        const int img_bytes = g.H * g.W * g.C * 4;
        const __amdgpu_buffer_rsrc_t xrsrc =
            __builtin_amdgcn_make_buffer_rsrc(const_cast<float*>(X) + (size_t)img * g.H * g.W * g.C, 0, img_bytes, 0x00020000);
        const __amdgpu_buffer_rsrc_t drsrc =
            __builtin_amdgcn_make_buffer_rsrc(const_cast<float*>(dY) + (size_t)img * g.H * g.W * g.C, 0, img_bytes, 0x00020000);
        const int lane16 = lane * 16;
        const v4f zero4 = {0.f, 0.f, 0.f, 0.f};
        const float relu_lo = relu_in ? 0.f : -__builtin_inff();
        const v4f relu_lo4 = {relu_lo, relu_lo, relu_lo, relu_lo};
        const bool has_aff = in_scale != nullptr;
        v4f scq[TKB], shq[TKB];
#pragma unroll
        for (int kb = 0; kb < TKB; ++kb) {
            const int ch = (tk * TKB + kb) * 16 + (lane & 3) * 4;
            scq[kb] = has_aff ? *reinterpret_cast<const v4f*>(in_scale + ch) : (v4f){1.f, 1.f, 1.f, 1.f};
            shq[kb] = has_aff ? *reinterpret_cast<const v4f*>(in_shift + ch) : (v4f){0.f, 0.f, 0.f, 0.f};
        }
        v4f lv[KP][GPP];
        int dst[KP];
        int aff[KP], aff2[KP];
        const int rowstride = g.W * g.C * 4;
#define DAM_RW_REQUEST(XR0_, NX_, DR0_, ND_, LV_, DST_, KP_, AFF_)                                                  \
    do {                                                                                                                   \
        _Pragma("unroll") for (int k = 0; k < KP_; ++k) {                                                                  \
            const int pl_ = cwl + NL * k;                                                                          \
            const int nxp_ = (NX_) * TKB;                                                                                  \
            const bool isx_ = pl_ < nxp_;                                                                                  \
            const int q_ = isx_ ? pl_ : pl_ - nxp_;                                                                        \
            const int i_ = isx_ ? q_ / TKB : q_ / TNB, c_ = isx_ ? q_ - i_ * TKB : q_ - i_ * TNB;                          \
            const int row_ = (isx_ ? (XR0_) : (DR0_)) + i_;                                                                \
            const bool need_ = isx_ ? row_ <= r_end : (i_ < (ND_) && row_ < r_end);                                        \
            const bool inimg_ = need_ && row_ >= 0 && row_ < g.H;                                                          \
            const int rel_ = row_ - r_begin + 1;                                            \
            const int xi_ = rw_mod<RW_NRX>(rel_);                                                                          \
            const int di_ = (row_ - r_begin) & (RW_NRD - 1);                                                               \
            const int ldsoff_ = isx_ ? XBASE + c_ * XPLANE + xi_ * ROWB : DBASE + c_ * DPLANE + di_ * ROWB;                \
            const int chan_ = isx_ ? (tk * TKB + c_) * 64 : (tn * TNB + c_) * 64;                                          \
            const int soff_ = (inimg_ ? row_ : 0) * rowstride + chan_;                                                     \
            if (isx_) {                                                                                                    \
                _Pragma("unroll") for (int gi = 0; gi < GPP; ++gi)                                                         \
                    LV_[k][gi] = __builtin_bit_cast(v4f, __builtin_amdgcn_raw_buffer_load_b128(xrsrc, loffb[gi], soff_, 0)); \
            } else {                                                                                                       \
                _Pragma("unroll") for (int gi = 0; gi < GPP; ++gi)                                                         \
                    LV_[k][gi] = __builtin_bit_cast(v4f, __builtin_amdgcn_raw_buffer_load_b128(drsrc, loffb[gi], soff_, 0)); \
            }                                                                                                              \
            DST_[k] = need_ ? (ldsoff_ | (inimg_ ? 0 : 1 << 30)) : -1;                                                     \
            AFF_[k] = (isx_ && has_aff) ? c_ : (isx_ ? -1 : -2);                                                           \
        }                                                                                                                  \
    } while (0)
#define DAM_RW_WRITE(ADDR_, DATA_, GI_)                                                                                    \
    asm volatile("s_mov_b64 exec, %2\n\tds_write_b128 %0, %1 offset:%3\n\ts_mov_b64 exec, -1"                              \
                 : : "v"(ADDR_), "v"(DATA_), "s"(cmask[GI_]), "n"((GI_) * 1024) : "memory")
#define DAM_RW_COMMIT(LV_, DST_, KP_, AFF_)                                                                         \
    do {                                                                                                                   \
        _Pragma("unroll") for (int k = 0; k < KP_; ++k) {                                                                  \
            if (DST_[k] >= 0) {                                                                                            \
                const int va_ = lane16 + (DST_[k] & 0x3fffffff);                                                           \
                if (DST_[k] >> 30) {                                                                                       \
                    _Pragma("unroll") for (int gi = 0; gi < GPP; ++gi) DAM_RW_WRITE(va_, zero4, gi);                       \
                } else if (AFF_[k] >= 0) {                                                                                 \
                    const v4f sc_ = (TKB > 1 && AFF_[k] > 0) ? scq[TKB - 1] : scq[0];                                      \
                    const v4f sh_ = (TKB > 1 && AFF_[k] > 0) ? shq[TKB - 1] : shq[0];                                      \
                    _Pragma("unroll") for (int gi = 0; gi < GPP; ++gi) {                                                   \
                        v4f v_ = __builtin_elementwise_fma(LV_[k][gi], sc_, sh_);                                          \
                        v_ = __builtin_elementwise_max(v_, relu_lo4);                    \
                        DAM_RW_WRITE(va_, v_, gi);                                                                         \
                    }                                                                                                      \
                } else {                                                                                                   \
                    _Pragma("unroll") for (int gi = 0; gi < GPP; ++gi) DAM_RW_WRITE(va_, LV_[k][gi], gi);                  \
                }                                                                                                          \
            }                                                                                                              \
        }                                                                                                                  \
    } while (0)
        constexpr int KPB = (2 * TKB + NL - 1) / NL;
        v4f lvb[KPB][GPP], lv2[KP][GPP];
        int dstb[KPB], dst2[KP], affb[KPB];
        DAM_WSTAMP(9);
        DAM_RW_REQUEST(r_begin - 1, RPS, r_begin, RPS, lv, dst, KP, aff);
        DAM_RW_REQUEST(r_begin + RPS - 1, 2, r_begin, 0, lvb, dstb, KPB, affb);
        DAM_WSTAMP(10);
        DAM_RW_ZERO();
        DAM_WSTAMP(11);
        DAM_RW_COMMIT(lv, dst, KP, aff);
        DAM_RW_COMMIT(lvb, dstb, KPB, affb);
        DAM_WSTAMP(12);
        asm volatile("s_waitcnt lgkmcnt(0)\n\ts_barrier" ::: "memory");
#define DAM_RW_SLOT(T_, LV_, DST_, AFF_) DAM_RW_REQUEST(r_begin + RPS * (T_) + 1, RPS, r_begin + RPS * (T_), RPS, LV_, DST_, KP, AFF_)
        DAM_WSTAMP(2);
        DAM_RW_SLOT(1, lv, dst, aff);
        DAM_RW_SLOT(2, lv2, dst2, aff2);
        for (int s = 0; s < n_slots2; s += 2) {
            DAM_RW_COMMIT(lv, dst, KP, aff);
            DAM_RW_SLOT(s + 3, lv, dst, aff);
            DAM_WSTAMP(5);
            asm volatile("s_waitcnt lgkmcnt(0)\n\ts_barrier" ::: "memory");
            DAM_WSTAMP(7);
            DAM_RW_COMMIT(lv2, dst2, KP, aff2);
            DAM_RW_SLOT(s + 4, lv2, dst2, aff2);
            DAM_WSTAMP(5);
            asm volatile("s_waitcnt lgkmcnt(0)\n\ts_barrier" ::: "memory");
            DAM_WSTAMP(7);
        }
#undef DAM_RW_SLOT
#undef DAM_RW_REQUEST
#undef DAM_RW_WRITE
#undef DAM_RW_COMMIT
    } else {
        const int cw = wave;
        const int lane_b = kq * 64 + j * 4;
        DAM_RW_ZERO();
        asm volatile("s_waitcnt lgkmcnt(0)\n\ts_barrier" ::: "memory");
        DAM_WSTAMP(2);
#define DAM_RW_SCHED()                                                                                                     \
    do {                                                                                                                   \
        _Pragma("unroll") for (int i_ = 0; i_ < 8; ++i_) {                                                                 \
            __builtin_amdgcn_sched_group_barrier(0x008, NL == 4 ? 2 : 1, 0);                                               \
            __builtin_amdgcn_sched_group_barrier(0x100, 1, 0);                                                             \
        }                                                                                                                  \
        __builtin_amdgcn_sched_group_barrier(0x008, 9 * TNB * TKB, 0);                                                     \
        __builtin_amdgcn_sched_barrier(0);                                                                                 \
    } while (0)
#define DAM_RW_LOAD(T_, BUF_)                                                                                              \
    do {                                                                                                                   \
        _Pragma("unroll") for (int nb = 0; nb < TNB; ++nb)                                                                 \
            av[BUF_][nb] = *reinterpret_cast<const float*>(smem + vd[nb] + (T_) * 256);                                    \
        _Pragma("unroll") for (int kb = 0; kb < TKB; ++kb)                                                                 \
            _Pragma("unroll") for (int a = 0; a < 3; ++a)                                                                  \
                _Pragma("unroll") for (int b = 0; b < 3; ++b)                                                              \
                    bv[BUF_][kb][a * 3 + b] = *reinterpret_cast<const float*>(smem + vx[kb][a] + ((T_) * 256 + b * 64));   \
    } while (0)
#define DAM_RW_ROW(F_, RW_, PART_, SUB_)                       \
    do {                                                                                                                   \
        int vx[TKB][3], vd[TNB];                                                                                           \
        _Pragma("unroll") for (int a = 0; a < 3; ++a) {                                                                    \
            const int xi = rw_mod<RW_NRX>(RPS * s + (RW_) + a);                 \
            _Pragma("unroll") for (int kb = 0; kb < TKB; ++kb) vx[kb][a] = lane_b + (XBASE - 64 + kb * XPLANE + xi * ROWB + (PART_)); \
        }                                                                                                                  \
        _Pragma("unroll") for (int nb = 0; nb < TNB; ++nb)                                                                 \
            vd[nb] = lane_b + (DBASE + nb * DPLANE + ((RPS * s + (RW_)) & (RW_NRD - 1)) * ROWB + (PART_));                 \
        float av[2][TNB], bv[2][TKB][9];                                                                                   \
        constexpr int NS_ = (STEPS + (F_) - 1) / (F_);                                                                     \
        DAM_RW_LOAD(0, 0);                                                                                                 \
        _Pragma("unroll") for (int t = 0; t < NS_; ++t) {                                                                  \
            if ((F_) > 1 && (SUB_) + (F_) * t >= STEPS) break;                 \
            if (t + 1 < NS_) DAM_RW_LOAD((F_) * (t + 1), (t + 1) & 1);                                                     \
            _Pragma("unroll") for (int nb = 0; nb < TNB; ++nb)                                                             \
                _Pragma("unroll") for (int kb = 0; kb < TKB; ++kb)                                                         \
                    _Pragma("unroll") for (int tap = 0; tap < 9; ++tap) {                                                  \
                        const int idx = (nb * TKB + kb) * 9 + tap;                                                         \
                        acc[idx] = __builtin_amdgcn_mfma_f32_16x16x4f32(av[t & 1][nb], bv[t & 1][kb][tap], acc[idx], 0, 0, 0); \
                    }                                                                                                      \
            DAM_RW_SCHED();                                                                                                \
        }                                                                                                                  \
    } while (0)
        for (int s = 0; s < n_slots2; ++s) {
            const int rows_here = r_end - (r_begin + RPS * s);
            if (HV == 1 && TNB * TKB == 1 && rows_here == 1) {
                DAM_RW_ROW(4, 0, cw * 256, cw);
            } else {
                const int rw = cw / HV, half = cw - rw * HV;
                if (rw < rows_here) DAM_RW_ROW(1, rw, half * STEPS * 256, 0);
            }
            DAM_WSTAMP(5);
            asm volatile("s_waitcnt lgkmcnt(0)\n\ts_barrier" ::: "memory");
            DAM_WSTAMP(7);
        }
    }
#undef DAM_RW_ROW
#undef DAM_RW_LOAD
#undef DAM_RW_SCHED

    __syncthreads();
    float* red = reinterpret_cast<float*>(smem);
    for (int w = 0; w < 4; ++w) {
        if (wave == w) {
#pragma unroll
            for (int i = 0; i < NBLK; ++i) {
                float4* d4 = reinterpret_cast<float4*>(red + (i * 64 + lane) * 4);
                if (w == 0) {
                    *d4 = make_float4(acc[i].x, acc[i].y, acc[i].z, acc[i].w);
                } else {
                    float4 o = *d4;
                    o.x += acc[i].x; o.y += acc[i].y; o.z += acc[i].z; o.w += acc[i].w;
                    *d4 = o;
                }
            }
        }
        __syncthreads();
    }
    float4* out = reinterpret_cast<float4*>(partial) + ((size_t)by * gridDim.x + bx) * NBLK * 64;
#ifdef DAM_WGR_STAMPS
    DAM_WSTAMP(8);
    if (lane == 0 && (wave == 0 || wave == 4)) {
        unsigned long long* sp = reinterpret_cast<unsigned long long*>(out) + (wave >> 2) * 32;
        for (int i = 0; i < 32; ++i) sp[i] = stamp_v[i];
    }
#else
    for (int e = tid; e < NBLK * 64; e += (256 + 64 * NL)) out[e] = reinterpret_cast<const float4*>(red)[e];
#endif
}

#undef DAM_RW_ZERO

template <int TNB, int TKB, int STEPS, int KP, int GPP, int HV = 1, int NL = 8>
int launch_wgrad_rows(int B, int H, int W, int C, const float* X, const float* dY, const float* in_scale, const float* in_shift,
                      int relu_in, float* partial, int64_t ws_floats, float* dw, int n_real, int k_real, void* queue,
                      hipStream_t st) {
    constexpr int NBLK = TNB * TKB * 9;
    RowsGeo g;
    g.B = B; g.H = H; g.W = W; g.C = C;
    constexpr int RPS = 4 / HV, NRX = 2 * RPS + 2, NRD = 2 * RPS;
    g.P4 = ((W + 2 + 4 * HV - 1) / (4 * HV)) * (4 * HV);
    if (g.P4 != STEPS * 4 * HV) return DAM_ERR_UNSUPPORTED;
    g.gpp = (g.P4 * 64 + 1023) / 1024;
    if (g.gpp > GPP || (RPS * (TKB + TNB) + NL - 1) / NL > KP) return DAM_ERR_UNSUPPORTED;
    const int nblk = C / 16;
    if (nblk % TNB || nblk % TKB || H >= 8000) return DAM_ERR_UNSUPPORTED;
    const int tiles_n = nblk / TNB;
    g.tiles_k = nblk / TKB;
    const int nx = tiles_n * g.tiles_k;
    const size_t rowb = (size_t)g.P4 * 64;
    size_t lds = RW_GUARD + (size_t)TKB * NRX * rowb + (size_t)TNB * NRD * rowb + RW_TAIL;
    if (lds < (size_t)NBLK * 1024) lds = (size_t)NBLK * 1024;
    if (lds > 160 * 1024) return DAM_ERR_UNSUPPORTED;
    auto strips = [&](int per_cu) { const int w = 256 * per_cu / (nx * B); return w > 0 ? w : 1; };
    int spi = strips(1);
    if (nx * B * spi < 205 && lds * 2 <= 160 * 1024) spi = strips(2);
    if (spi > (int)cdiv(H, RPS)) spi = (int)cdiv(H, RPS);
    if (spi > H) spi = H;
    for (;; --spi) {
        g.spi = spi;
        g.rps = (int)cdiv(H, spi);
        if ((int64_t)B * g.spi * nx * NBLK * 256 <= ws_floats || spi == 1) break;
    }
    const int nsplit = B * g.spi;
    if ((int64_t)nsplit * nx * NBLK * 256 > ws_floats) return DAM_ERR_WORKSPACE;
    if (!raise_lds_limit<&wgrad_rows_kernel<TNB, TKB, STEPS, KP, GPP, HV, NL>>(160 * 1024)) return DAM_ERR_LAUNCH;
    hipLaunchKernelGGL((wgrad_rows_kernel<TNB, TKB, STEPS, KP, GPP, HV, NL>), dim3(nx, nsplit), dim3((256 + 64 * NL)), lds, st, g, X, dY, in_scale,
                       in_shift, relu_in, partial);
    DAM_CHECK_LAUNCH();
    return reduce_submit(queue, partial, dw, nsplit, nx, TNB, TKB, 3, 3, n_real, k_real, 3, 3, 1, g.tiles_k, st);
}

struct RowsS2Geo {
    int B, H, W, C;
    int Ho, Wo, N;
    int rps, spi;
    int tiles_k;
};
template <> __device__ __forceinline__ int rw_mod<18>(int v) { return v - ((v * 58255) >> 20) * 18; }

template <int TNB, int STEPS, int KP, int GPPX, int GPPD, int HV>
__global__ __launch_bounds__(RW_THREADS) void wgrad_rows_s2_kernel(const RowsS2Geo g, const float* __restrict__ X,
                                                                   const float* __restrict__ dY, float* __restrict__ partial) {
    extern __shared__ __attribute__((aligned(16))) unsigned char smem[];
    constexpr int NBLK = TNB * 9;
    constexpr int RPS = 4 / HV, NRX = 4 * RPS + 2, NRD = 2 * RPS;
    constexpr int P4 = STEPS * 4 * HV;
    constexpr int XROWB = 2 * P4 * 64, DROWB = P4 * 64;
    constexpr int XPLANE = NRX * XROWB, DPLANE = NRD * DROWB;
    constexpr int XBASE = RW_GUARD, DBASE = XBASE + XPLANE;
    constexpr int lds_bytes = DBASE + TNB * DPLANE + RW_TAIL;
    constexpr int NXP = 2 * RPS;
    constexpr int GPP = GPPX > GPPD ? GPPX : GPPD;
    const int tid = threadIdx.x, lane = tid & 63;
    const int wave = __builtin_amdgcn_readfirstlane(tid >> 6);
    const int j = lane & 15, kq = lane >> 4;
    int bx = blockIdx.x, by = blockIdx.y;
    {
        const int nxg = gridDim.x, L = blockIdx.y * nxg + blockIdx.x, full = (gridDim.y >> 3) << 3;
        if (L < full * nxg) { const int c = L & 7, r = L >> 3; bx = r % nxg; by = (r / nxg) * 8 + c; }
    }
    const int tn = bx / g.tiles_k, tk = bx - tn * g.tiles_k;
    const int img = by / g.spi, sidx = by - img * g.spi;
    const int r_begin = (int)(((long long)sidx * g.Ho) / g.spi), r_end = (int)(((long long)(sidx + 1) * g.Ho) / g.spi);
    const int n_slots = (r_end - r_begin + RPS - 1) / RPS;
    const int n_slots2 = (n_slots + 1) & ~1;

#define DAM_RW_ZERO()                                                                                                      \
    do {                                                                                                                   \
        for (int e = tid * 16; e < lds_bytes; e += RW_THREADS * 16)                                                        \
            *reinterpret_cast<float4*>(smem + e) = make_float4(0.f, 0.f, 0.f, 0.f);                                        \
        asm volatile("s_waitcnt lgkmcnt(0)\n\ts_barrier" ::: "memory");                                                    \
    } while (0)

    v4f acc[NBLK];
#pragma unroll
    for (int i = 0; i < NBLK; ++i) acc[i] = (v4f){0.f, 0.f, 0.f, 0.f};

    if (wave >= 4) {
        const int cwl = wave - 4;
        int loffb[KP][GPP];
        unsigned long long cmask[KP][GPP];
#pragma unroll
        for (int k = 0; k < KP; ++k) {
            const bool isx = cwl + RW_LOADERS * k < NXP;
#pragma unroll
            for (int gi = 0; gi < GPP; ++gi) {
                const int L = gi * 64 + lane, e = L >> 2, quad = L & 3;
                const int col = isx ? (e < P4 ? 2 * e - 1 : 2 * (e - P4)) : e;
                const int lim = isx ? g.W : g.Wo, cells = isx ? 2 * P4 : P4;
                const bool ok = e < cells && col >= 0 && col < lim;
                const int colc = col < 0 ? 0 : (col >= lim ? lim - 1 : col);
                loffb[k][gi] = (colc * (isx ? g.C : g.N) + quad * 4) * 4;
                cmask[k][gi] = __ballot(ok);
            }
        }
        const int ximg_bytes = g.H * g.W * g.C * 4, dimg_bytes = g.Ho * g.Wo * g.N * 4;
        const __amdgpu_buffer_rsrc_t xrsrc =
            __builtin_amdgcn_make_buffer_rsrc(const_cast<float*>(X) + (size_t)img * g.H * g.W * g.C, 0, ximg_bytes, 0x00020000);
        const __amdgpu_buffer_rsrc_t drsrc =
            __builtin_amdgcn_make_buffer_rsrc(const_cast<float*>(dY) + (size_t)img * g.Ho * g.Wo * g.N, 0, dimg_bytes, 0x00020000);
        const int lane16 = lane * 16;
        const v4f zero4 = {0.f, 0.f, 0.f, 0.f};
        const int xrowstride = g.W * g.C * 4, drowstride = g.Wo * g.N * 4;
        const int x_first = 2 * r_begin - 1, x_last = 2 * r_end - 1;
        v4f lv[KP][GPP], lv2[KP][GPP], lvb[GPPX];
        int dst[KP], dst2[KP], dstb;
#define DAM_RW2_REQUEST(XR0_, DR0_, LV_, DST_)                                                                             \
    do {                                                                                                                   \
        _Pragma("unroll") for (int k = 0; k < KP; ++k) {                                                                   \
// ... 411 lines not shown
        PendingTile& p = q->pend;
        constexpr int sig = TNB | TKB << 4 | TA << 8 | TB << 12;
        if (p.njobs > 0 && (p.sig != sig || memcmp(&p.g, &g, sizeof(WgradGeo)) != 0 || p.njobs == WG_MAX_JOBS)) {
            const int rc = p.launch(q, st);
            if (rc != DAM_OK) return rc;
        }
        const int i = p.njobs++;
        p.sig = sig; p.g = g; p.launch = &launch_pending_tile<TNB, TKB, TA, TB>;
        p.jobs.X[i] = X; p.jobs.dY[i] = dY; p.jobs.sc[i] = sc; p.jobs.sh[i] = sh; p.jobs.partial[i] = partial;
        p.jobs.relu_in[i] = relu_in;
        p.dw[i] = dw; p.ws_floats[i] = ws_floats; p.n_real[i] = n_real; p.k_real[i] = k_real;
        return DAM_OK;
    }
    WgradJobs jobs;
    memset(&jobs, 0, sizeof(jobs));
    jobs.X[0] = X; jobs.dY[0] = dY; jobs.sc[0] = sc; jobs.sh[0] = sh; jobs.partial[0] = partial; jobs.relu_in[0] = relu_in;
    return launch_wgrad_jobs<TNB, TKB, TA, TB>(g, jobs, 1, ws_floats, &dw, &n_real, &k_real, queue, st);
}

}
}

extern "C" int64_t dam_wgrad_queue_bytes(void) { return (int64_t)sizeof(dam::WgradQueue); }

extern "C" int dam_wgrad_queue_init(void* queue) {
    if (!queue) return DAM_ERR_BAD_ARG;
    dam::WgradQueue* q = static_cast<dam::WgradQueue*>(queue);
    const int batching = q->magic == dam::WGRAD_QUEUE_MAGIC ? q->batching : 0;
    memset(q, 0, sizeof(*q));
    q->magic = dam::WGRAD_QUEUE_MAGIC;
    q->batching = batching;
    return DAM_OK;
}

extern "C" int dam_wgrad_queue_set_batching(void* queue, int on) {
    dam::WgradQueue* q = static_cast<dam::WgradQueue*>(queue);
    if (!q || q->magic != dam::WGRAD_QUEUE_MAGIC) return DAM_ERR_BAD_ARG;
    if (q->pend.njobs > 0 || q->pend_direct.jobs.njobs > 0) return DAM_ERR_BAD_ARG;
    q->batching = on ? 1 : 0;
    return DAM_OK;
}

extern "C" int dam_wgrad_queue_pending(const void* queue) {
    const dam::WgradQueue* q = static_cast<const dam::WgradQueue*>(queue);
    return q && q->magic == dam::WGRAD_QUEUE_MAGIC ? q->batch.njobs + q->pend.njobs + q->pend_direct.jobs.njobs : -1;
}

extern "C" int dam_wgrad_queue_flush(void* queue, void* stream) {
    dam::WgradQueue* q = static_cast<dam::WgradQueue*>(queue);
    if (!q || q->magic != dam::WGRAD_QUEUE_MAGIC) return DAM_ERR_BAD_ARG;
    if (q->pend.njobs > 0) {
        const int rc = q->pend.launch(q, (hipStream_t)stream);
        if (rc != DAM_OK) return rc;
    }
    if (q->pend_direct.jobs.njobs > 0) {
        const int rc = q->pend_direct.launch(q, (hipStream_t)stream);
        if (rc != DAM_OK) return rc;
    }
    return dam::reduce_flush(q->batch, (hipStream_t)stream);
}

extern "C" int64_t dam_conv2d_wgrad_workspace_floats(int n_out, int c_in, int kh, int kw) {
    if (n_out <= 0 || c_in <= 0 || kh <= 0 || kw <= 0) return 0;
    const int64_t whole = dam::cdiv(n_out, 32) * dam::cdiv(c_in, 32) * 4 * 256 * (int64_t)kh * kw;
    const int64_t a = 512LL * 36 * 256 + 4 * whole;
    return a;
}

extern "C" int dam_conv2d_wgrad_f32(const float* x, int B, int H, int W, int C, int in_nchw, const float* in_scale,
                                    const float* in_shift, int relu_in, const float* dy, int Ho, int Wo, int n_chan,
                                    int n_out, int kh, int kw, int stride, int pad, int dil, float* dw, int c_real,
                                    float* workspace, int64_t workspace_floats, void* reduce_queue, void* stream) {
    using namespace dam;
    if (!x || !dy || !dw || !workspace || B <= 0 || H <= 0 || W <= 0 || C <= 0 || Ho <= 0 || Wo <= 0) return DAM_ERR_BAD_ARG;
    if (c_real < 0 || c_real > C) return DAM_ERR_BAD_ARG;
    const int k_real = c_real ? c_real : C;
    if (n_chan % 16 || n_out > n_chan || (stride != 1 && stride != 2)) return DAM_ERR_UNSUPPORTED;
    if (in_nchw ? C > 16 : C % 16) return DAM_ERR_UNSUPPORTED;
    if (in_scale && !in_shift) return DAM_ERR_BAD_ARG;
    hipStream_t st = (hipStream_t)stream;
    if (kh == 3 && kw == 3 && stride == 1 && pad == 1 && dil == 1 && !in_nchw && Ho == H && Wo == W && C == n_chan) {
        int rc = DAM_ERR_UNSUPPORTED;
#define DAM_WGR(...) launch_wgrad_rows<__VA_ARGS__>(B, H, W, C, x, dy, in_scale, in_shift, relu_in, workspace, workspace_floats, dw, n_out, k_real, reduce_queue, st)
        if (C == 16) { rc = DAM_WGR(1, 1, 33, 1, 9); if (rc == DAM_ERR_UNSUPPORTED) rc = DAM_WGR(1, 1, 28, 1, 14, 2); }
        else if (W > 80) rc = DAM_WGR(2, 1, 14, 1, 7, 2);
        else if (W > 48) { rc = DAM_WGR(2, 1, 17, 2, 5); if (rc == DAM_ERR_UNSUPPORTED) rc = DAM_WGR(2, 1, 14, 2, 4); }
        else if (W > 20) rc = DAM_WGR(2, 1, 9, 2, 3);
        else if (W > 12) rc = DAM_WGR(2, 1, 5, 3, 2, 1, 4);
        else if (W > 6) rc = DAM_WGR(2, 1, 3, 2, 1);
#undef DAM_WGR
        if (rc != DAM_ERR_UNSUPPORTED) return rc;
    }
#define DAM_WGD(TN_, TK_, KH_, KW_) \
    launch_wgrad_direct<TN_, TK_, KH_, KW_>(B, H, W, C, Ho, Wo, n_chan, stride, pad, dil, x, dy, workspace, workspace_floats, dw, n_out, k_real, reduce_queue, st)
    if (kh == 1 && kw == 1 && pad == 0 && !in_nchw && !in_scale) {
        int rc = DAM_WGD(2, 2, 1, 1);
        if (rc == DAM_ERR_UNSUPPORTED) rc = DAM_WGD(2, 1, 1, 1);
        if (rc == DAM_ERR_UNSUPPORTED) rc = DAM_WGD(1, 1, 1, 1);
        if (rc != DAM_ERR_UNSUPPORTED) return rc;
    }
    if (kh == 3 && kw == 3 && !in_nchw && !in_scale && stride == 2 && pad == 1 && dil == 1) {
#define DAM_WGR2(...) launch_wgrad_rows_s2<__VA_ARGS__>(B, H, W, C, Ho, Wo, n_chan, x, dy, workspace, workspace_floats, dw, n_out, k_real, reduce_queue, st)
        int rc = DAM_ERR_UNSUPPORTED;
        if (Wo > 56) rc = DAM_WGR2(2, 9, 1, 9, 5, 2);
        else if (Wo > 34) rc = DAM_WGR2(2, 7, 1, 7, 4, 2);
        else if (Wo > 28) rc = DAM_WGR2(2, 9, 2, 5, 3, 1);
        else if (Wo > 18) rc = DAM_WGR2(2, 7, 2, 4, 2, 1);
        else if (Wo > 14) rc = DAM_WGR2(2, 5, 2, 3, 2, 1);
#undef DAM_WGR2
        if (rc != DAM_ERR_UNSUPPORTED) return rc;
    }
    if (kh == 3 && kw == 3 && !in_nchw && !in_scale && Wo >= 16 && stride == 2) {
        int rc = DAM_WGD(2, 1, 3, 3);
        if (rc == DAM_ERR_UNSUPPORTED) rc = DAM_WGD(1, 1, 3, 3);
        if (rc != DAM_ERR_UNSUPPORTED) return rc;
    }
#undef DAM_WGD
    WgradGeo g;
    memset(&g, 0, sizeof(g));
    g.B = B; g.H = H; g.W = W; g.C = C; g.Ho = Ho; g.Wo = Wo; g.N = n_chan; g.s = stride; g.KH = kh; g.KW = kw;
    g.off_h = -pad; g.step_h = dil; g.off_w = -pad; g.step_w = dil;
    g.r0 = -pad; g.c0 = -pad;
    g.PWin = (Wo - 1) * stride + (kw - 1) * dil + 1;
    g.PWs = (int)cdiv(g.PWin, stride);
    g.PWT = g.PWs * stride;
    const int ta_rows = (kh == 3 && kw == 3) ? 3 : 1;
    auto set_tile = [&](int tmw_max) {
        const int64_t npix_ = (int64_t)Ho * Wo, parts_ = cdiv(npix_, tmw_max);
        const int tmw = (int)(cdiv(cdiv(npix_, parts_), 16) * 16);
        int rows_out = (tmw + Wo - 2) / Wo + 1;
        if (rows_out > Ho) rows_out = Ho;
        g.TMW = tmw;
        g.PR = (rows_out - 1) * stride + (ta_rows - 1) * dil + 1;
        g.tiles_m = (int)cdiv((int64_t)Ho * Wo, tmw);
        g.total_tiles = g.tiles_m * B;
    };
    auto lds_bytes = [&](int tnb, int tkb) { return (size_t)tkb * g.PR * g.PWT * 64 + (size_t)tnb * g.TMW * 64; };
    g.nchunks = in_nchw ? 1 : C / 16;
    g.nblk = n_chan / 16;
    g.in_nchw = in_nchw; g.relu_in = relu_in;
    int tnb = 2, tkb = 2;
    if (kh == 5 && kw == 5 && g.nblk == 3 && g.nchunks % 2 == 0) { tnb = 3; tkb = 2; }
    bool small = g.nchunks == 1 || g.nblk == 1;
    set_tile(256);
    if (!small && lds_bytes(tnb, tkb) > 72 * 1024) {
        set_tile(128);
        if (lds_bytes(tnb, tkb) > 72 * 1024) {
            if (tnb == 2 && tkb == 2) small = true;
            else { tnb = tkb = 2; set_tile(256); if (lds_bytes(2, 2) > 72 * 1024) { set_tile(128); if (lds_bytes(2, 2) > 72 * 1024) small = true; } }
        }
    }
    if (small) {
        set_tile(256);
        if (lds_bytes(1, 1) > 72 * 1024) set_tile(128);
    }
#define DAM_WG(TN_, TK_, TA_, TB_) \
    return launch_wgrad<TN_, TK_, TA_, TB_>(g, x, dy, in_scale, in_shift, workspace, workspace_floats, dw, n_out, k_real, reduce_queue, st)
    if (kw == 3 && kh == 3) { if (small) DAM_WG(1, 1, 3, 3); else DAM_WG(2, 2, 3, 3); }
    if (kw == 1 && kh == 1) { if (small) DAM_WG(1, 1, 1, 1); else DAM_WG(2, 2, 1, 1); }
    if (kw == 5) { if (small) DAM_WG(1, 1, 1, 5); else if (tnb == 3) DAM_WG(3, 2, 1, 5); else DAM_WG(2, 2, 1, 5); }
    if (kw == 7) { if (small) DAM_WG(1, 1, 1, 7); else DAM_WG(2, 2, 1, 7); }
    if (kw == 9) { if (small) DAM_WG(1, 1, 1, 9); else DAM_WG(2, 2, 1, 9); }
#undef DAM_WG
    return DAM_ERR_UNSUPPORTED;
}
```

### deep-audio-mixer_amd/layers.py

```python
import torch
import torch.nn as nn

from . import ops


def _slot(p):
    return None if p is None else getattr(p, '_dam_grad', None)


class ConvSpec:

    def __init__(self, cin, cout, k, stride=1, pad=0, dil=1, in_nchw=False):
        self.cin, self.cout, self.k, self.stride, self.pad, self.dil, self.in_nchw = cin, cout, k, stride, pad, dil, in_nchw
        self.wp = self.wpt = None
        self.nhwc16 = None
        if in_nchw and k == 3 and stride == 1 and pad == 1 and dil == 1 and cin <= 16:
            self.nhwc16 = _Nhwc16Spec(self)

    def packed(self, w, transpose=False):
        cached = self.wpt if transpose else self.wp
        return cached if cached is not None else ops.pack_weights(w, transpose=transpose)

    def fwd(self, x, w, bias=None):
        return ops.conv2d_fwd(x, self.packed(w), self.cout, self.k, self.k, self.stride, self.pad, self.dil,
                              bias=bias, in_nchw=self.in_nchw)

    def fwd_conv(self, x, w, bn, training, bias=None, in_affine=None, fuse_stats=True, finalize=True):
        wp = self.packed(w)
        aff = {} if in_affine is None else dict(in_scale=in_affine[0], in_shift=in_affine[1], relu_in=True)
        if training and not self.in_nchw and fuse_stats:
            n16 = (self.cout + 15) // 16 * 16
            buf = ops.bn_partial_buffer(x.device, n16)
            c, parts, out4 = ops.conv2d_fwd(x, wp, self.cout, self.k, self.k, self.stride, self.pad, self.dil, bias=bias,
                                            bn_partial=buf, bn=_bn_args(bn, training), finalize=finalize, **aff)
            if not finalize:
                return c, ((buf, parts) if parts > 0 else None)
            return c, ((out4[0], out4[1], out4[2], out4[3]) if parts > 0 else None)
        return ops.conv2d_fwd(x, wp, self.cout, self.k, self.k, self.stride, self.pad, self.dil, bias=bias,
                              in_nchw=self.in_nchw, **aff), None

    def fwd_bn(self, x, w, bn, training, bias=None, in_affine=None):
        c, stats = self.fwd_conv(x, w, bn, training, bias=bias, in_affine=in_affine)
        return (c,) + tuple(stats if stats is not None else _bn_fwd_stats(c, bn, training))

    def fwd_bn_apply(self, x, w, bn, training, in_affine=None, res=None, res_affine=None, sign_bits=False, bias=None):
        rs, rh = res_affine if res_affine is not None else (None, None)
        if training:
            c, rec = self.fwd_conv(x, w, bn, training, bias=bias, in_affine=in_affine, finalize=False)
            rec = rec if rec is not None else ops.bn_stats_partial(c)
            (m, i, sc, sh), out = ops.bn_finalize_apply(rec[0], rec[1], _bn_args(bn, training), c, relu=True, res=res,
                                                        res_scale=rs, res_shift=rh, sign_bits=sign_bits)
            return c, m, i, sc, sh, out
        c, m, i, sc, sh = self.fwd_bn(x, w, bn, training, bias=bias, in_affine=in_affine)
        return c, m, i, sc, sh, ops.bn_apply(c, sc, sh, relu=True, res=res, res_scale=rs, res_shift=rh, sign_bits=sign_bits)

    def wgrad(self, x, dy, in_affine=None, out=None):
        aff = {} if in_affine is None else dict(in_scale=in_affine[0], in_shift=in_affine[1], relu_in=True)
        return ops.conv2d_wgrad(x, dy, self.cout, self.k, self.k, self.stride, self.pad, self.dil,
                                in_nchw=self.in_nchw, out=out, defer=out is not None, **aff)

    def dgrad(self, dy, w, hw, **kw):
        return ops.conv2d_dgrad(dy, self.packed(w, transpose=True), self.cin, hw[0], hw[1], self.k, self.k,
                                self.stride, self.pad, self.dil, **kw)


class _Nhwc16Spec(ConvSpec):

    def __init__(self, parent):
        self.cin, self.cout, self.k, self.stride, self.pad, self.dil, self.in_nchw = 16, parent.cout, 3, 1, 1, 1, False
        self.parent, self.nhwc16, self.wpt = parent, None, None

    @property
    def wp(self):
        return self.parent.wp

    def packed(self, w, transpose=False):
        return self.parent.packed(w, transpose)

    def wgrad(self, x, dy, in_affine=None, out=None):
        return ops.conv2d_wgrad(x, dy, self.cout, 3, 3, 1, 1, 1, out=out, c_real=self.parent.cin, defer=out is not None)


class WeightPacker:

    def __init__(self, pairs):
        self.pairs = list(pairs)
        self._key = None

    def _build(self):
        rows, dev = [], self.pairs[0][1].device
        L = ops._lib.lib()
        for spec, w, need_t in self.pairs:
            o, i, kh, kw = w.shape
            for transpose in ((False, True) if need_t else (False,)):
                n_out, k_in = (i, o) if transpose else (o, i)
                n = L.dam_conv_packed_weight_count(n_out, k_in, kh, kw)
                buf = torch.empty(n, dtype=torch.float32, device=dev)
                if transpose:
                    spec.wpt = buf
                else:
                    spec.wp = buf
                rows.append([w.data_ptr(), buf.data_ptr(), o, i, kh, kw, int(transpose), n])
        self.desc = torch.tensor(rows, dtype=torch.int64).to(dev)
        self.n, self.max_total = len(rows), max(r[7] for r in rows)

    def pack_all(self):
        key = tuple(w.data_ptr() for _, w, _ in self.pairs)
        if key != self._key:
            self._build()
            self._key = key
        ops.pack_weights_multi(self.desc, self.n, self.max_total)


def _bn_args(bn, training):
    mom = bn.momentum if bn.momentum is not None else 0.1
    track = training and bn.track_running_stats
    return (bn.weight, bn.bias, bn.running_mean if track else None, bn.running_var if track else None,
            bn.num_batches_tracked if track else None, mom, bn.eps)


def _bn_fwd_stats(c, bn, training):
    if training or bn.running_mean is None:
        return ops.bn_stats(c, *_bn_args(bn, training))
    return ops.bn_eval_affine(bn.weight, bn.bias, bn.running_mean, bn.running_var, bn.eps)


def _hw(x, in_nchw):
    return (x.shape[2], x.shape[3]) if in_nchw else (x.shape[1], x.shape[2])


class FoldedConvBn:

    def __init__(self, spec, conv, bn):
        self.spec, self.conv, self.bn = spec, conv, bn
        self._key = self.wp = self.bias = None

    def foldable(self):
        return self.bn.running_mean is not None and self.bn.running_var is not None

    def _tensors(self):
        bn, conv = self.bn, self.conv
        return [t for t in (conv.weight, conv.bias, bn.weight, bn.bias, bn.running_mean, bn.running_var) if t is not None]

    def get(self):
        key = (ops.PARAM_EPOCH,) + tuple((t.data_ptr(), t._version) for t in self._tensors())
        if key != self._key:
            bn, conv = self.bn, self.conv
            with torch.no_grad():
                scale = bn.weight * torch.rsqrt(bn.running_var + bn.eps)
                shift = bn.bias - bn.running_mean * scale
                if conv.bias is not None:
                    shift = shift + conv.bias * scale
                n16 = (self.spec.cout + 15) // 16 * 16
# ... 418 lines not shown
```

### deep-audio-mixer_amd/ops.py

```python
import collections
import ctypes
import numbers
import os

import torch

from . import _lib


def _f32c(t, name):
    if t is None:
        return None
    if t.dtype != torch.float32 or not t.is_contiguous():
        raise ValueError('%s must be a contiguous float32 tensor' % name)
    return t


def conv_out_size(n, k, stride=1, pad=0, dil=1):
    return (n + 2 * pad - dil * (k - 1) - 1) // stride + 1


def pack_weights(w, transpose=False, out=None):
    _lib.require_cuda(w)
    w = _f32c(w.detach(), 'weight')
    o, i, kh, kw = w.shape
    n_out, k_in = (i, o) if transpose else (o, i)
    n = _lib.lib().dam_conv_packed_weight_count(n_out, k_in, kh, kw)
    if out is None:
        out = torch.empty(n, dtype=torch.float32, device=w.device)
    _lib.check(_lib.lib().dam_conv_pack_weights_f32(_lib.ptr(w), o, i, kh, kw, 1 if transpose else 0,
                                                    _lib.ptr(out), _lib.stream()), 'dam_conv_pack_weights_f32')
    return out


def pack_weights_multi(desc, n_tensors, max_total):
    _lib.check(_lib.lib().dam_conv_pack_weights_multi_f32(_lib.ptr(desc), n_tensors, max_total, _lib.stream()),
               'dam_conv_pack_weights_multi_f32')


DGRAD_S2 = not os.environ.get('DAM_NO_DGRAD_S2')
dgrad_s2_launches = 0
DGRAD_BN_SUMS = not os.environ.get('DAM_NO_DGRAD_SUMS')


def _bn_fin_struct(bn, out4):
    gamma, beta, rm, rv, nbt, mom, eps = bn
    return _lib.BnFin(_lib.ptr(gamma), _lib.ptr(beta), _lib.ptr(rm), _lib.ptr(rv), _lib.ptr(nbt), float(mom), float(eps),
                      _lib.ptr(out4[0]), _lib.ptr(out4[1]), _lib.ptr(out4[2]), _lib.ptr(out4[3]))


def _tapgrid(x, B, H, W, C, in_nchw, wp, k_chunks, n_out, bias, in_scale, in_shift, relu_in, y, OHt, OWt, Ho, Wo,
             out_stride, oo_h, oo_w, in_stride, nA, nB, off_h, step_h, off_w, step_w, wt_base, wt_sa, wt_sb,
             res=None, res_mask=None, bn_partial=None, relu_out=False, batch=None, bn_bwd=None):
    parts = ctypes.c_int(0)
    ws = _workspace(y.device, min(8 * y.numel(), 8 * 400 * 64 * 64))
    st = _lib.lib().dam_conv2d_tapgrid_f32(
        _lib.ptr(x), B, H, W, C, 1 if in_nchw else 0, _lib.ptr(wp), k_chunks, n_out, _lib.ptr(bias),
        _lib.ptr(in_scale), _lib.ptr(in_shift), 1 if relu_in else 0, 1 if relu_out else 0, _lib.ptr(y), OHt, OWt, Ho, Wo,
        out_stride,
        oo_h, oo_w, in_stride, nA, nB, off_h, step_h, off_w, step_w, wt_base, wt_sa, wt_sb, _lib.ptr(res),
        _lib.ptr(res_mask), _lib.ptr(bn_partial), ctypes.byref(parts) if bn_partial is not None else None,
        ctypes.byref(bn_bwd) if bn_bwd is not None else None,
        _lib.ptr(ws), ws.numel(),
        ctypes.addressof(batch) if batch is not None else None, _lib.stream())
    _lib.check(st, 'dam_conv2d_tapgrid_f32')
    return parts.value


def conv2d_fwd(x, wp, n_out, kh, kw, stride=1, pad=0, dil=1, bias=None, in_scale=None, in_shift=None,
               relu_in=False, in_nchw=False, bn_partial=None, bn=None, res=None, relu_out=False, finalize=True, out=None):
    _lib.require_cuda(x, wp)
    _f32c(x, 'x'), _f32c(bias, 'bias'), _f32c(in_scale, 'in_scale'), _f32c(in_shift, 'in_shift'), _f32c(res, 'res')
    if in_nchw:
        B, C, H, W = x.shape
        k_chunks = 1
    else:
        B, H, W, C = x.shape
        k_chunks = C // 16
    n16 = (n_out + 15) // 16 * 16
    Ho, Wo = conv_out_size(H, kh, stride, pad, dil), conv_out_size(W, kw, stride, pad, dil)
    if Ho <= 0 or Wo <= 0:
        raise ValueError('convolution output would be empty')
    if out is None:
        y = torch.empty((B, Ho, Wo, n16), dtype=torch.float32, device=x.device)
    else:
        if out.dtype != torch.float32 or not out.is_contiguous() or tuple(out.shape) != (B, Ho, Wo, n16) or out.device != x.device:
            raise ValueError('out must be a contiguous float32 tensor of shape %s on %s' % ((B, Ho, Wo, n16), x.device))
        y = out
    parts = _tapgrid(x, B, H, W, C, in_nchw, wp, k_chunks, n16, bias, in_scale, in_shift, relu_in, y, Ho, Wo, Ho, Wo,
                     1, 0, 0, stride, kh, kw, -pad, dil, -pad, dil, 0, kw, 1, res=res, bn_partial=bn_partial,
                     relu_out=relu_out)
    if bn is not None and bn_partial is not None:
        out4 = bn_finalize(bn_partial, parts, *bn) if parts > 0 and finalize else None
        return y, parts, out4
    if bn_partial is not None:
        return y, parts
    return y


CONV_FAMILIES = ('none', 'strip', 'pipe', 'pipe_ranges', 'tile', 'tile_batch', '1x1')
ConvLaunch = collections.namedtuple('ConvLaunch', 'family MB NB NCH T33 LW EPI SO PU STATS KS ksplit ranges')


def conv_last_launch():
    v = (ctypes.c_int * 16)()
    _lib.check(_lib.lib().dam_conv_last_launch(v), 'dam_conv_last_launch')
    return ConvLaunch(CONV_FAMILIES[v[0]], *v[1:13])


def _dgrad_axis(parity, pad, dil, k, stride):
    valid = [t for t in range(k) if (parity + pad - t * dil) % stride == 0]
    if not valid:
        return None
    k0 = valid[0]
    kstep = valid[1] - valid[0] if len(valid) > 1 else 1
    return len(valid), k0, kstep, (parity + pad - k0 * dil) // stride, -(kstep * dil) // stride


def conv2d_dgrad(dy, wpt, n_in, H, W, kh, kw, stride=1, pad=0, dil=1, res=None, res_mask=None, accumulate_into=None,
                 bn_bwd=None, res_mask_bits=None, pair_1x1=None, _s2_sums=None):
    _lib.require_cuda(dy, wpt)
    if bn_bwd is not None and stride == 2:
        if accumulate_into is not None or res is not None or len(bn_bwd) < 6 or bn_bwd[5] is None or bn_bwd[3] is not None:
            raise ValueError('bn_bwd at stride 2: mask as sign bytes, no residual / accumulation')
        xb, mean, invstd, up_bits = bn_bwd[0], bn_bwd[1], bn_bwd[2], bn_bwd[5]
        _lib.require_cuda(xb)
        n16 = (n_in + 15) // 16 * 16
        if tuple(xb.shape) != (dy.shape[0], H, W, n16):
            raise ValueError('bn_bwd: x has the shape of the data gradient')
        rec = torch.empty(_lib.lib().dam_bn_workspace_floats(n16), dtype=torch.float32, device=dy.device)
        epi = _lib.BnBwdSums(_lib.ptr(xb), _lib.ptr(mean), _lib.ptr(invstd), None, None, None, _lib.ptr(up_bits))
        got = conv2d_dgrad(dy, wpt, n_in, H, W, kh, kw, stride, pad, dil, pair_1x1=pair_1x1, _s2_sums=(epi, rec))
        return got if isinstance(got, tuple) else (got, None)
    if bn_bwd is not None:
        if stride != 1 or accumulate_into is not None:
            raise ValueError('bn_bwd: stride-1 data gradients only')
        if res is not None and (res_mask is None or res_mask_bits is None):
            raise ValueError('bn_bwd with a residual: res_mask and res_mask_bits')
        _f32c(dy, 'dy'), _f32c(res, 'res'), _f32c(res_mask, 'res_mask')
        xb, mean, invstd, msc, msh = bn_bwd[:5]
        up_bits = bn_bwd[5] if len(bn_bwd) > 5 else None
        if (up_bits is None) == (msc is None) or (up_bits is not None and res is None):
            raise ValueError('bn_bwd: the mask as (scale, shift) or -- with a residual -- as sign bytes')
        _lib.require_cuda(xb)
        B, Ho, Wo, Co = dy.shape
        n16 = (n_in + 15) // 16 * 16
        if tuple(xb.shape) != (B, H, W, n16):
            raise ValueError('bn_bwd: x has the shape of the data gradient')
        dx = torch.empty((B, H, W, n16), dtype=torch.float32, device=dy.device)
        rec = torch.empty(_lib.lib().dam_bn_workspace_floats(n16), dtype=torch.float32, device=dy.device)
        epi = _lib.BnBwdSums(_lib.ptr(xb), _lib.ptr(mean), _lib.ptr(invstd), _lib.ptr(msc), _lib.ptr(msh), _lib.ptr(res_mask_bits),
                             _lib.ptr(up_bits))
        parts = _tapgrid(dy, B, Ho, Wo, Co, False, wpt, Co // 16, n16, None, None, None, False, dx, H, W, H, W, 1, 0, 0, 1,
                         kh, kw, pad, -dil, pad, -dil, 0, kw, 1, res, res_mask, bn_partial=rec, bn_bwd=epi)
        return dx, ((rec, parts) if parts > 0 else None)
    _f32c(dy, 'dy'), _f32c(res, 'res'), _f32c(res_mask, 'res_mask')
    B, Ho, Wo, Co = dy.shape
    n16 = (n_in + 15) // 16 * 16
    if accumulate_into is not None:
        dx, res, res_mask = accumulate_into, accumulate_into, None
    else:
        dx = torch.empty((B, H, W, n16), dtype=torch.float32, device=dy.device)
    if stride == 1:
        _tapgrid(dy, B, Ho, Wo, Co, False, wpt, Co // 16, n16, None, None, None, False, dx, H, W, H, W, 1, 0, 0, 1,
                 kh, kw, pad, -dil, pad, -dil, 0, kw, 1, res, res_mask)
        return dx
    if pair_1x1 is not None:
        dy2, wpt2 = pair_1x1
        _lib.require_cuda(dy2, wpt2)
        _f32c(dy2, 'pair dy')
        if accumulate_into is not None or res is not None or tuple(dy2.shape) != tuple(dy.shape):
            raise ValueError('pair_1x1: a second gradient of the same shape, no residual / accumulation')
        a0 = _dgrad_axis(0, pad, dil, kh, stride), _dgrad_axis(0, pad, dil, kw, stride)
        if a0[0] is None or a0[1] is None or a0[0][0] != 1 or a0[1][0] != 1 or a0[0][3] != 0 or a0[1][3] != 0:
            raise ValueError('pair_1x1: class (0, 0) of this operator is not a single tap at offset 0')
    if (DGRAD_S2 and stride == 2 and kh == 3 and kw == 3 and pad == 1 and dil == 1 and accumulate_into is None and res is None
            and Ho == (H + 1) // 2 and Wo == (W + 1) // 2):
        parts = ctypes.c_int(0)
        st = _lib.lib().dam_dgrad_s2_3x3_f32(_lib.ptr(dy), _lib.ptr(wpt), _lib.ptr(pair_1x1[0]) if pair_1x1 else None,
                                             _lib.ptr(pair_1x1[1]) if pair_1x1 else None, B, Ho, Wo, Co, n16, _lib.ptr(dx), H, W,
                                             ctypes.byref(_s2_sums[0]) if _s2_sums else None,
                                             _lib.ptr(_s2_sums[1]) if _s2_sums else None, ctypes.byref(parts) if _s2_sums else None,
                                             _lib.stream())
        if st == 0:
            global dgrad_s2_launches
            dgrad_s2_launches += 1
            if _s2_sums:
                return dx, ((_s2_sums[1], parts.value) if parts.value > 0 else None)
            return dx
        if st != -2:
# ... 865 lines not shown
```

### include/dam_hip.h

```cpp
#ifndef DAM_HIP_H
#define DAM_HIP_H

#include <stdint.h>

#ifdef __cplusplus
extern "C" {
#endif

typedef enum dam_status {
    DAM_OK = 0,
    DAM_ERR_BAD_ARG = -1,
    DAM_ERR_UNSUPPORTED = -2,
    DAM_ERR_LAUNCH = -3,
    DAM_ERR_WORKSPACE = -4
} dam_status;

typedef enum dam_pcm_dtype { DAM_PCM_F32 = 0, DAM_PCM_F64 = 1, DAM_PCM_S16 = 2, DAM_PCM_S32 = 3 } dam_pcm_dtype;
#define DAM_PCM_INDIRECT 0x100
#define DAM_PCM_ROTATE 0x200
struct dam_bn_bwd_sums;

#define DAM_ABI_VERSION 26
const char* dam_arch(void);
int dam_abi_version(void);

int dam_host_dontfork_pinned(int64_t* n_mappings_host, int64_t* n_bytes_host);

int dam_step_mark_create(void** mark_host);
int dam_step_mark_record(void* mark, void* stream);
int dam_step_mark_wait(void* mark, void* stream);
int dam_step_mark_synchronize(void* mark);
int dam_step_mark_destroy(void* mark);


int64_t dam_stft_twiddle_count(int n_fft);
int dam_stft_fill_twiddles_host(int n_fft, float* table_host );

int dam_stft_logmag_f32(const void* pcm, int pcm_dtype, int64_t n_tracks, int64_t n_samples, int channels,
                        int64_t pcm_track_stride, const float* window, const float* twiddles,
                        const float* gain, int n_fft, int hop, float amin, int normalize,
                        float* out, void* stream);

int dam_stft_logmag_strided_f32(const void* pcm, int pcm_dtype, int64_t n_outer, int64_t outer_stride, int64_t n_inner,
                                int64_t inner_stride, int64_t n_samples, int channels, int64_t sample_stride,
                                int64_t channel_stride, const float* window, const float* twiddles, const float* gain,
                                int n_fft, int hop, float amin, int normalize, float* out, float* out_tail, int n_tail,
                                void* stream);

int dam_stft_complex_f32(const void* pcm, int pcm_dtype, int64_t n_tracks, int64_t n_samples, int channels,
                         int64_t pcm_track_stride, int64_t n_sum, int64_t sum_stride, const float* window,
                         const float* twiddles, const float* gain, int n_fft, int hop, float* out, void* stream);
int dam_stft_complex_strided_f32(const void* pcm, int pcm_dtype, int64_t n_outer, int64_t outer_stride, int64_t n_inner,
                                 int64_t inner_stride, int64_t n_sum, int64_t sum_stride, int64_t n_samples, int channels,
                                 int64_t sample_stride, int64_t channel_stride, const float* window, const float* twiddles,
                                 const float* gain, int n_fft, int hop, float* out, void* stream);
int64_t dam_istft_workspace_bytes(int64_t n_tracks, int64_t n_frames, int n_fft, int hop, int64_t length);
int dam_istft_f32(const float* spec, const float* mag_db, int64_t n_tracks, int64_t n_frames, int n_fft, int hop,
                  int64_t length, const float* window, const float* twiddles, float* out, void* workspace,
                  int64_t workspace_bytes, void* stream);

int dam_augment_gains_f32(uint64_t seed, const int64_t* items, int64_t first_item, int n_items, int n_tracks,
                          float lo, float hi, float* gains, void* stream);


int64_t dam_conv_packed_weight_count(int n_out, int k_in, int kh, int kw);

int dam_conv_pack_weights_f32(const float* w_oihw, int O, int I, int KH, int KW, int transpose,
                              float* packed, void* stream);

int dam_conv_pack_weights_multi_f32(const int64_t* desc_dev, int n_tensors, int64_t max_total, void* stream);

int dam_conv2d_tapgrid_f32(const float* x, int B, int H, int W, int C, int in_nchw, const float* w_packed,
                           int k_chunks, int n_out, const float* bias, const float* in_scale,
                           const float* in_shift, int relu_in, int relu_out, float* y, int OHt, int OWt, int Ho, int Wo,
                           int out_stride, int out_off_h, int out_off_w, int in_stride, int nA, int nB,
                           int off_h, int step_h, int off_w, int step_w, int wt_base, int wt_sa, int wt_sb,
                           const float* res, const float* res_mask, float* bn_partial, int* bn_parts_host,
                           const struct dam_bn_bwd_sums* bn_bwd, float* workspace, int64_t workspace_floats,
                           void* batch, void* stream);

int dam_conv1x1_pair_f32(const float* x1, const float* w1_packed, int tap1, const float* x2, const float* w2_packed, int tap2,
                         int B, int H, int W, int C, int n_out, float* y, int OHt, int OWt, int out_stride, int out_off_h,
                         int out_off_w, void* stream);

int dam_dgrad_s2_3x3_f32(const float* dy, const float* w_packed_t, const float* dy_pair, const float* w_pair_packed_t, int B,
                         int Hd, int Wd, int Co, int Ci, float* dx, int H, int W, const struct dam_bn_bwd_sums* bn_bwd,
                         float* bn_partial, int* bn_parts_host, void* stream);

int dam_conv_s2_pair_fwd_f32(const float* x, const float* w_packed, const float* wsc_packed, int B, int H, int W, int Ci, int Co,
                             float* y, float* ysc, float* partial, float* partial_sc, int* parts_host, void* stream);

int64_t dam_conv_batch_bytes(void);
int dam_conv_batch_init(void* batch);
int dam_conv_batch_flush(void* batch, void* stream);

int dam_conv_last_launch(int* out16_host);

int64_t dam_conv2d_wgrad_workspace_floats(int n_out, int c_in, int kh, int kw);
int dam_conv2d_wgrad_f32(const float* x, int B, int H, int W, int C, int in_nchw, const float* in_scale,
                         const float* in_shift, int relu_in, const float* dy, int Ho, int Wo, int n_chan,
                         int n_out, int kh, int kw, int stride, int pad, int dil, float* dw, int c_real,
                         float* workspace, int64_t workspace_floats, void* reduce_queue, void* stream);

int64_t dam_wgrad_queue_bytes(void);
int dam_wgrad_queue_init(void* queue);
int dam_wgrad_queue_pending(const void* queue);
int dam_wgrad_queue_flush(void* queue, void* stream);
int dam_wgrad_queue_set_batching(void* queue, int on);

int dam_strip_diag_counters(uint32_t* out2_host, int reset);

int64_t dam_bn_workspace_floats(int C);

typedef struct dam_bn_fin {
    const float* gamma; const float* beta;
    float* running_mean; float* running_var; int64_t* num_batches_tracked;
    float momentum, eps;
    float* save_mean; float* save_invstd; float* scale; float* shift;
} dam_bn_fin;

typedef struct dam_bn_bwd_sums {
    const float* x; const float* mean; const float* invstd; const float* mask_scale; const float* mask_shift;
    const uint8_t* res_mask_bits;
    const uint8_t* mask_bits;
} dam_bn_bwd_sums;

int dam_bn_stats_f32(const float* x, int64_t n_pixels, int C, const float* gamma, const float* beta,
                     float* running_mean, float* running_var, int64_t* num_batches_tracked,
                     float momentum, float eps, float* save_mean, float* save_invstd, float* scale,
                     float* shift, float* workspace, void* stream);

int dam_bn_stats_pair_f32(const float* x_a, const float* x_b, int64_t n_pixels, int C, const struct dam_bn_fin* a,
                          const struct dam_bn_fin* b, float* workspace, void* stream);

int dam_bn_finalize_f32(const float* partial, int parts, int C, const float* gamma, const float* beta,
                        float* running_mean, float* running_var, int64_t* num_batches_tracked,
                        float momentum, float eps, float* save_mean, float* save_invstd, float* scale,
                        float* shift, void* stream);

int dam_bn_finalize_pair_f32(const float* partial_a, const float* partial_b, int parts, int C, const struct dam_bn_fin* a,
                             const struct dam_bn_fin* b, void* stream);

int dam_bn_stats_partial_f32(const float* x, int64_t n_pixels, int C, float* workspace, int* parts_host, void* stream);

int dam_bn_finalize_apply_f32(const float* partial, int parts, int C, const struct dam_bn_fin* fin, const float* x,
                              int64_t n_pixels, const float* res, const float* res_scale, const float* res_shift, int relu,
                              float* y, uint8_t* sign_bits, void* stream);

int dam_bn_eval_affine_f32(int C, const float* gamma, const float* beta, const float* running_mean,
                           const float* running_var, float eps, float* save_mean, float* save_invstd,
                           float* scale, float* shift, void* stream);

int dam_bn_apply_f32(const float* x, int64_t n_pixels, int C, const float* scale, const float* shift,
                     const float* res, const float* res_scale, const float* res_shift, int relu, float* y,
                     uint8_t* sign_bits, void* stream);
// ... 132 lines not shown
```

Baseline: 2.030 million stem-spectrogram-frames/s.

## Add paired-tap stem path for conv with few real input channels

Threads the real input channel count (c_real) through the tapgrid conv API so the stem conv, whose input is padded to 16 channels but has at most 8 real ones, can use a STEM kernel variant. In forward, the strip kernel packs two 3x3 taps into one 16-channel MFMA step (5 items instead of 9), with fillers doubled up. The weight-gradient rows kernel gets a matching STEM specialization. Together these avoid multiplying zero-padded channels, at the cost of more template variants and more intricate LDS indexing.

```diff
diff --git a/deep-audio-mixer_amd/_lib.py b/deep-audio-mixer_amd/_lib.py
--- a/deep-audio-mixer_amd/_lib.py
+++ b/deep-audio-mixer_amd/_lib.py
@@ -7,7 +7,7 @@
 _HERE = os.path.dirname(os.path.abspath(__file__))
 LIB_PATH = os.environ.get('DAM_LIB_PATH') or os.path.join(_HERE, 'libdam_hip.so')
 
-EXPECTED_ABI = 26
+EXPECTED_ABI = 27
 
 _STATUS = {0: 'DAM_OK', -1: 'DAM_ERR_BAD_ARG', -2: 'DAM_ERR_UNSUPPORTED', -3: 'DAM_ERR_LAUNCH',
            -4: 'DAM_ERR_WORKSPACE'}
@@ -38,7 +38,7 @@
     'dam_conv_packed_weight_count': (c_i64, [c_i, c_i, c_i, c_i]),
     'dam_conv_pack_weights_f32': (c_i, [c_p, c_i, c_i, c_i, c_i, c_i, c_p, c_p]),
     'dam_conv_pack_weights_multi_f32': (c_i, [c_p, c_i, c_i64, c_p]),
-    'dam_conv2d_tapgrid_f32': (c_i, [c_p, c_i, c_i, c_i, c_i, c_i, c_p, c_i, c_i, c_p, c_p, c_p, c_i, c_i, c_p] +
+    'dam_conv2d_tapgrid_f32': (c_i, [c_p, c_i, c_i, c_i, c_i, c_i, c_i, c_p, c_i, c_i, c_p, c_p, c_p, c_i, c_i, c_p] +
                                [c_i] * 17 + [c_p, c_p, c_p, c_p, c_p, c_p, c_i64, c_p, c_p]),
     'dam_conv_batch_bytes': (c_i64, []),
     'dam_conv_batch_init': (c_i, [c_p]),
diff --git a/deep-audio-mixer_amd/csrc/dam_conv.hip b/deep-audio-mixer_amd/csrc/dam_conv.hip
--- a/deep-audio-mixer_amd/csrc/dam_conv.hip
+++ b/deep-audio-mixer_amd/csrc/dam_conv.hip
@@ -537,7 +537,7 @@
 extern "C" int dam_conv_last_launch(int* out16_host) {
     if (!out16_host) return DAM_ERR_BAD_ARG;
     const dam::ConvLaunchNote& n = dam::conv_last_launch;
-    const int v[16] = {n.family, n.MB, n.NB, n.NCH, n.T33, n.LW, n.EPI, n.SO, n.PU, n.STATS, n.KS, n.ksplit, n.ranges, 0, 0, 0};
+    const int v[16] = {n.family, n.MB, n.NB, n.NCH, n.T33, n.LW, n.EPI, n.SO, n.PU, n.STATS, n.KS, n.ksplit, n.ranges, n.STEM, 0, 0};
     for (int i = 0; i < 16; ++i) out16_host[i] = v[i];
     return DAM_OK;
 }
@@ -558,7 +558,7 @@
     return dam::conv_batch_flush(*b, (hipStream_t)stream);
 }
 
-extern "C" int dam_conv2d_tapgrid_f32(const float* x, int B, int H, int W, int C, int in_nchw, const float* w_packed,
+extern "C" int dam_conv2d_tapgrid_f32(const float* x, int B, int H, int W, int C, int c_real, int in_nchw, const float* w_packed,
                                       int k_chunks, int n_out, const float* bias, const float* in_scale,
                                       const float* in_shift, int relu_in, int relu_out, float* y, int OHt, int OWt, int Ho, int Wo,
                                       int out_stride, int out_off_h, int out_off_w, int in_stride, int nA, int nB,
@@ -583,6 +583,7 @@
     if (n_out % 16 || (in_stride != 1 && in_stride != 2) || out_stride < 1) return DAM_ERR_UNSUPPORTED;
     if (in_nchw ? (C > 16 || k_chunks != 1) : (C % 16 || k_chunks != C / 16)) return DAM_ERR_UNSUPPORTED;
     if (in_scale && !in_shift) return DAM_ERR_BAD_ARG;
+    if (c_real < 0 || c_real > C) return DAM_ERR_BAD_ARG;
     if (B > 65535) return DAM_ERR_UNSUPPORTED;
     ConvGeo g;
     g.B = B; g.H = H; g.W = W; g.C = C; g.Ho = Ho; g.Wo = Wo; g.N = n_out; g.OHt = OHt; g.OWt = OWt;
@@ -591,6 +592,7 @@
     g.wt_base = wt_base; g.wt_sa = wt_sa; g.wt_sb = wt_sb;
     g.in_nchw = in_nchw; g.relu_in = relu_in; g.relu_out = relu_out != 0; g.nchunks = k_chunks; g.NBtot = n_out / 16;
     g.epi_bwd = 0;
+    g.c_real = c_real == C ? 0 : c_real;
     const int h_lo = off_h + (step_h < 0 ? (nA - 1) * step_h : 0), h_hi = off_h + (step_h > 0 ? (nA - 1) * step_h : 0);
     const int w_lo = off_w + (step_w < 0 ? (nB - 1) * step_w : 0), w_hi = off_w + (step_w > 0 ? (nB - 1) * step_w : 0);
     g.r0 = h_lo; g.c0 = w_lo;
diff --git a/deep-audio-mixer_amd/csrc/dam_conv_geo.h b/deep-audio-mixer_amd/csrc/dam_conv_geo.h
--- a/deep-audio-mixer_amd/csrc/dam_conv_geo.h
+++ b/deep-audio-mixer_amd/csrc/dam_conv_geo.h
@@ -24,6 +24,7 @@
     int ksplit;
     int gps;
     int epi_bwd;
+    int c_real;
 };
 
 struct BnBwdEpi {
@@ -46,7 +47,7 @@
 enum ConvFamily { CONV_FAM_NONE = 0, CONV_FAM_STRIP = 1, CONV_FAM_PIPE = 2, CONV_FAM_PIPE_RANGES = 3, CONV_FAM_TILE = 4,
                   CONV_FAM_TILE_BATCH = 5, CONV_FAM_1X1 = 6 };
 struct ConvLaunchNote {
-    int family, MB, NB, NCH, T33, LW, EPI, SO, PU, STATS, KS, ksplit, ranges;
+    int family, MB, NB, NCH, T33, LW, EPI, SO, PU, STATS, KS, ksplit, ranges, STEM;
 };
 extern thread_local ConvLaunchNote conv_last_launch;
 
diff --git a/deep-audio-mixer_amd/csrc/dam_conv_strip.hip b/deep-audio-mixer_amd/csrc/dam_conv_strip.hip
--- a/deep-audio-mixer_amd/csrc/dam_conv_strip.hip
+++ b/deep-audio-mixer_amd/csrc/dam_conv_strip.hip
@@ -91,7 +91,7 @@
     }
 }
 
-template <int MB, int NB, int NCH, bool T33, bool LW, int EPI, int SO>
+template <int MB, int NB, int NCH, bool T33, bool LW, int EPI, int SO, bool STEM = false>
 __global__ __launch_bounds__(SO ? 512 : STRIP_THREADS, 1) void conv_strip_kernel(const ConvGeo g, const StripGeo sg, const float* __restrict__ X,
                                                          const float4* __restrict__ Wp, const float* __restrict__ bias,
                                                          float* __restrict__ Y, const float* __restrict__ res,
@@ -659,8 +659,14 @@
         if (grp == 0) {
             constexpr bool ST = EPI == 0 && SO == 2, BIAS = EPI == 0 && (SO == 3 || SO == 4), RADD = EPI == 0 && SO == 4,
                            RMSK = EPI == 0 && SO == 5, NEED_R = EPI != 0 || RADD || RMSK;
-            constexpr int NI = 9 * NCH;
-            static_assert(NI >= 2 * MB + 1, "one filler per item: MB write-out units, MB geometry units, the operand prefetch");
+            static_assert(!STEM || (NCH == 1 && NB == 1 && !LW), "the paired-tap form: one 16-channel chunk, one output block");
+            constexpr int NI = STEM ? 5 : 9 * NCH;
+            constexpr int FPI = STEM ? 2 : 1;
+            static_assert(FPI * (NI - 1) >= 2 * MB - 1 && (STEM || NI >= 2 * MB + 1), "fillers: MB write-out units, MB geometry units");
+            const bool k_up = STEM && kq >= 2;
+            const int lane_xs = lane_x + (k_up ? 32 : 0);
+            const int w_lane_p = w_lane + (k_up ? 1024 - 512 : 0), w_lane_r = w_lane + (k_up ? 3 * 1024 - 512 : 0);
+            int baseX3[2][STEM ? MB : 1], baseX4[2][STEM ? MB : 1];
             v4f accX[2][MB][NB];
             int voffX[2][MB];
             int baseX[2][3][MB];
@@ -700,17 +706,30 @@
         SO_TAG_CHECK(qa_, MBI_);                                                                                          \
         const bool nx_ = j >= qa_.y;                                                                                      \
         voffX[P_][MBI_] = (nx_ ? lane_oD : lane_o) + qa_.x;                                                               \
-        baseX[P_][0][MBI_] = lane_x + (nx_ ? qb_.y : qa_.z);                                                              \
-        baseX[P_][1][MBI_] = lane_x + (nx_ ? qb_.z : qa_.w);                                                              \
-        baseX[P_][2][MBI_] = lane_x + (nx_ ? qb_.w : qb_.x);                                                              \
+        baseX[P_][0][MBI_] = lane_xs + (nx_ ? qb_.y : qa_.z);                                                             \
+        baseX[P_][1][MBI_] = lane_xs + (nx_ ? qb_.z : qa_.w);                                                             \
+        baseX[P_][2][MBI_] = lane_xs + (nx_ ? qb_.w : qb_.x);                                                             \
+        if constexpr (STEM) {                                                                                             \
+            baseX3[P_][MBI_] = k_up ? baseX[P_][1][MBI_] + 64 : baseX[P_][0][MBI_] + 128;                                 \
+            baseX4[P_][MBI_] = baseX[P_][2][MBI_] + (k_up ? 96 : 128);                                                    \
+        }                                                                                                                 \
     } while (0)
 #define SO_LOAD(P_, I_, BUF_)                                                                                             \
     do {                                                                                                                  \
         constexpr int a_ = (I_) / (3 * NCH), b_ = ((I_) / NCH) % 3, cc_ = (I_) % NCH;                                     \
-        _Pragma("unroll") for (int nb = 0; nb < NB; ++nb)                                                                 \
-            wa[BUF_][nb] = *reinterpret_cast<const float4*>(smem + w_lane + ((((a_ * 3 + b_) * NCH + cc_) * NB + nb) * 1024)); \
-        _Pragma("unroll") for (int mb = 0; mb < MB; ++mb)                                                                 \
-            xv[BUF_][mb] = *reinterpret_cast<const float4*>(smem + (cc_ ? baseX[P_][a_][mb] + CHB : baseX[P_][a_][mb]) + b_ * 64); \
+        if constexpr (STEM) {                             \
+            constexpr int ar_ = (I_) < 3 ? (I_) : 0;                                                                      \
+            wa[BUF_][0] = *reinterpret_cast<const float4*>(                                                               \
+                smem + ((I_) < 3 ? w_lane_p + (I_) * 3 * 1024 : ((I_) == 3 ? w_lane_r + 2 * 1024 : w_lane + 8 * 1024)));  \
+            _Pragma("unroll") for (int mb = 0; mb < MB; ++mb)                                                             \
+                xv[BUF_][mb] = *reinterpret_cast<const float4*>(                                                          \
+                    smem + ((I_) < 3 ? baseX[P_][ar_][mb] : ((I_) == 3 ? baseX3[P_][mb] : baseX4[P_][mb])));              \
+        } else {                                                                                                          \
+            _Pragma("unroll") for (int nb = 0; nb < NB; ++nb)                                                             \
+                wa[BUF_][nb] = *reinterpret_cast<const float4*>(smem + w_lane + ((((a_ * 3 + b_) * NCH + cc_) * NB + nb) * 1024)); \
+            _Pragma("unroll") for (int mb = 0; mb < MB; ++mb)                                                             \
+                xv[BUF_][mb] = *reinterpret_cast<const float4*>(smem + (cc_ ? baseX[P_][a_][mb] + CHB : baseX[P_][a_][mb]) + b_ * 64); \
+        }                                                                                                                 \
     } while (0)
 #define SO_MFMA(P_, I_, BUF_)                                                                                             \
     do {                                                                                                                  \
@@ -791,17 +810,26 @@
             if constexpr (ST) ++st_n;                                                                                     \
         }                                                                                                                 \
     } while (0)
+#define SO_FILL1(P_, SA_, F_, WO_)                                                                                        \
+    do {                                                                                                                  \
+        if constexpr ((F_) < MB) {                                                                                        \
+            if constexpr (WO_) SO_UNIT(1 - (P_), (SA_) - 1, ((F_) < MB ? (F_) : 0), 0);                                   \
+            SO_TABREAD((SA_) + 1, ((F_) < MB ? (F_) : 0));                                                                \
+            SO_PREFETCH1(P_, ((F_) < MB ? (F_) : 0));                                                                     \
+        } else if constexpr ((F_) < 2 * MB) SO_GEOM(1 - (P_), ((F_) < 2 * MB && (F_) >= MB ? (F_) - MB : 0));             \
+    } while (0)
 #define SO_FILL(P_, S_, I_, WO_)                                                                                          \
     do {                                                                                                                  \
           \
          \
         int sa_ = (S_);                                                                                                   \
         asm volatile("" : "+s"(sa_));                                                                                     \
-        if constexpr ((I_) < MB) {                                                                                        \
-            if constexpr (WO_) SO_UNIT(1 - (P_), sa_ - 1, ((I_) < MB ? (I_) : 0), 0);                                     \
-            SO_TABREAD(sa_ + 1, ((I_) < MB ? (I_) : 0));                                                                  \
-            SO_PREFETCH1(P_, ((I_) < MB ? (I_) : 0));                                                                     \
-        } else if constexpr ((I_) < 2 * MB) SO_GEOM(1 - (P_), ((I_) < 2 * MB && (I_) >= MB ? (I_) - MB : 0));             \
+        if constexpr (FPI == 1 || (I_) == 0) {                                                                            \
+            SO_FILL1(P_, sa_, I_, WO_);                                                                                   \
+        } else {                                                                                                          \
+            SO_FILL1(P_, sa_, 2 * (I_) - 1, WO_);                                                                         \
+            SO_FILL1(P_, sa_, 2 * (I_), WO_);                                                                             \
+        }                                                                                                                 \
     } while (0)
 #define SO_PATTERN()                                                                                                      \
     do {                                                                                                                  \
@@ -815,11 +843,13 @@
     } while (0)
 #define SO_ITEM(P_, S_, I_, WO_)                                                                                          \
     do {                                                                                                                  \
-        if constexpr ((I_) + 1 < NI) SO_LOAD(P_, ((I_) + 1 < NI ? (I_) + 1 : 0), ((I_) + 1) & 1);                         \
-        SO_MFMA(P_, I_, (I_) & 1);                                                                                        \
-        if constexpr ((I_) != 0) SO_FILL(P_, S_, I_, WO_);                                                                \
-        SO_PATTERN();                                                                                                     \
-        __builtin_amdgcn_sched_barrier(0);                                                                                \
+        if constexpr ((I_) < NI) {                                                                                        \
+            if constexpr ((I_) + 1 < NI) SO_LOAD(P_, ((I_) + 1 < NI ? (I_) + 1 : 0), ((I_) + 1) & 1);                     \
+            SO_MFMA(P_, I_, (I_) & 1);                                                                                    \
+            if constexpr ((I_) != 0) SO_FILL(P_, S_, I_, WO_);                                                            \
+            SO_PATTERN();                                                                                                 \
+            __builtin_amdgcn_sched_barrier(0);                                                                            \
+        }                                                                                                                 \
     } while (0)
 #define SO_SLOT(P_, S_, WO_)                                                                                              \
     do {                                                                                                                  \
@@ -883,6 +913,7 @@
 #undef SO_PREFETCH1
 #undef SO_UNIT
 #undef SO_FILL
+#undef SO_FILL1
 #undef SO_PATTERN
 #undef SO_ITEM
 #undef SO_SLOT
@@ -976,16 +1007,16 @@
 
 }
 
-template <int MB, int NB, int NCH, bool T33, bool LW = false, int EPI = 0, int SO = 0>
+template <int MB, int NB, int NCH, bool T33, bool LW = false, int EPI = 0, int SO = 0, bool STEM = false>
 static int launch_strip(ConvGeo& g, StripGeo& sg, size_t lds, const float* X, const float* Wp, const float* bias, float* Y,
                         const float* res, const float* res_mask, float* stats, const float* in_scale, const float* in_shift,
                         const BnBwdEpi& bwd, hipStream_t st) {
-    if (lds > 64 * 1024 && !raise_lds_limit<&conv_strip_kernel<MB, NB, NCH, T33, LW, EPI, SO>>(160 * 1024)) return DAM_ERR_LAUNCH;
+    if (lds > 64 * 1024 && !raise_lds_limit<&conv_strip_kernel<MB, NB, NCH, T33, LW, EPI, SO, STEM>>(160 * 1024)) return DAM_ERR_LAUNCH;
     dim3 grid((unsigned)sg.strips, (unsigned)cdiv(g.N / 16, NB), (unsigned)g.B);
-    hipLaunchKernelGGL((conv_strip_kernel<MB, NB, NCH, T33, LW, EPI, SO>), grid, dim3(SO ? 512 : STRIP_THREADS), lds, st, g, sg, X, reinterpret_cast<const float4*>(Wp), bias,
+    hipLaunchKernelGGL((conv_strip_kernel<MB, NB, NCH, T33, LW, EPI, SO, STEM>), grid, dim3(SO ? 512 : STRIP_THREADS), lds, st, g, sg, X, reinterpret_cast<const float4*>(Wp), bias,
                        Y, res, res_mask, stats, in_scale, in_shift, bwd);
     DAM_CHECK_LAUNCH();
-    conv_last_launch = ConvLaunchNote{CONV_FAM_STRIP, MB, NB, NCH, T33, LW, EPI, SO, 0, 0, 0, 1, 1};
+    conv_last_launch = ConvLaunchNote{CONV_FAM_STRIP, MB, NB, NCH, T33, LW, EPI, SO, 0, 0, 0, 1, 1, STEM};
     return DAM_OK;
 }
 
@@ -1075,6 +1106,8 @@
         } else if (bwd.x) {
             DAM_SO_CASE(1, 1);
         } else if (stats) {
+            if (!bias && !res && !g.relu_out && c16 && g.c_real > 0 && g.c_real <= 8 && !in_scale)
+                return launch_strip<4, 1, 1, true, false, 0, 2, true>(DAM_STRIP_ARGS);
             if (!bias && !res && !g.relu_out) DAM_SO_CASE(0, 2);
         } else if (res && res_mask) {
             if (!bias && !g.relu_out) DAM_SO_CASE(0, 5);
diff --git a/deep-audio-mixer_amd/csrc/dam_wgrad.hip b/deep-audio-mixer_amd/csrc/dam_wgrad.hip
--- a/deep-audio-mixer_amd/csrc/dam_wgrad.hip
+++ b/deep-audio-mixer_amd/csrc/dam_wgrad.hip
@@ -352,13 +352,15 @@
 constexpr int RW_THREADS = 256 + 64 * RW_LOADERS, RW_GUARD = 64, RW_TAIL = 1280;
 template <int D> __device__ __forceinline__ int rw_mod(int v) { return D == 10 ? v - ((v * 52429) >> 19) * 10 : v - ((v * 43691) >> 18) * 6; }
 
-template <int TNB, int TKB, int STEPS, int KP, int GPP, int HV, int NL>
+template <int TNB, int TKB, int STEPS, int KP, int GPP, int HV, int NL, bool STEM = false>
 __global__ __launch_bounds__(256 + 64 * NL) void wgrad_rows_kernel(const RowsGeo g, const float* __restrict__ X,
                                                                 const float* __restrict__ dY, const float* __restrict__ in_scale,
                                                                 const float* __restrict__ in_shift, int relu_in,
                                                                 float* __restrict__ partial) {
     extern __shared__ __attribute__((aligned(16))) unsigned char smem[];
-    constexpr int NBLK = TNB * TKB * 9;
+    static_assert(!STEM || (TNB == 1 && TKB == 1), "the paired-tap form is a one-block tile");
+    constexpr int NTAP = STEM ? 5 : 9;
+    constexpr int NBLK = TNB * TKB * NTAP, NBLK_OUT = TNB * TKB * 9;
     constexpr int RPS = 4 / HV, RW_NRX = 2 * RPS + 2, RW_NRD = 2 * RPS;
     const int tid = threadIdx.x, lane = tid & 63;
     const int wave = __builtin_amdgcn_readfirstlane(tid >> 6);
@@ -524,37 +526,48 @@
     } else {
         const int cw = wave;
         const int lane_b = kq * 64 + j * 4;
+        const int lane_x = lane_b + (STEM && j >= 8 ? 32 : 0);
         DAM_RW_ZERO();
         asm volatile("s_waitcnt lgkmcnt(0)\n\ts_barrier" ::: "memory");
         DAM_WSTAMP(2);
 #define DAM_RW_SCHED()                                                                                                     \
     do {                                                                                                                   \
-        _Pragma("unroll") for (int i_ = 0; i_ < 8; ++i_) {                                                                 \
+        _Pragma("unroll") for (int i_ = 0; i_ < NTAP - 1; ++i_) {                                                          \
             __builtin_amdgcn_sched_group_barrier(0x008, NL == 4 ? 2 : 1, 0);                                               \
             __builtin_amdgcn_sched_group_barrier(0x100, 1, 0);                                                             \
         }                                                                                                                  \
-        __builtin_amdgcn_sched_group_barrier(0x008, 9 * TNB * TKB, 0);                                                     \
+        __builtin_amdgcn_sched_group_barrier(0x008, NBLK, 0);                                                              \
         __builtin_amdgcn_sched_barrier(0);                                                                                 \
     } while (0)
 #define DAM_RW_LOAD(T_, BUF_)                                                                                              \
     do {                                                                                                                   \
         _Pragma("unroll") for (int nb = 0; nb < TNB; ++nb)                                                                 \
             av[BUF_][nb] = *reinterpret_cast<const float*>(smem + vd[nb] + (T_) * 256);                                    \
-        _Pragma("unroll") for (int kb = 0; kb < TKB; ++kb)                                                                 \
-            _Pragma("unroll") for (int a = 0; a < 3; ++a)                                                                  \
-                _Pragma("unroll") for (int b = 0; b < 3; ++b)                                                              \
-                    bv[BUF_][kb][a * 3 + b] = *reinterpret_cast<const float*>(smem + vx[kb][a] + ((T_) * 256 + b * 64));   \
+        if constexpr (STEM) {                                                                                              \
+            _Pragma("unroll") for (int a = 0; a < 3; ++a)                                             \
+                bv[BUF_][0][a] = *reinterpret_cast<const float*>(smem + vx[0][a] + (T_) * 256);                            \
+            bv[BUF_][0][3] = *reinterpret_cast<const float*>(smem + vx3 + (T_) * 256);                \
+            bv[BUF_][0][4] = *reinterpret_cast<const float*>(smem + vx[0][2] + ((T_) * 256 + 128));   \
+        } else {                                                                                                           \
+            _Pragma("unroll") for (int kb = 0; kb < TKB; ++kb)                                                             \
+                _Pragma("unroll") for (int a = 0; a < 3; ++a)                                                              \
+                    _Pragma("unroll") for (int b = 0; b < 3; ++b)                                                          \
+                        bv[BUF_][kb][a * 3 + b] = *reinterpret_cast<const float*>(smem + vx[kb][a] + ((T_) * 256 + b * 64)); \
+        }                                                                                                                  \
     } while (0)
 #define DAM_RW_ROW(F_, RW_, PART_, SUB_)                       \
     do {                                                                                                                   \
         int vx[TKB][3], vd[TNB];                                                                                           \
         _Pragma("unroll") for (int a = 0; a < 3; ++a) {                                                                    \
             const int xi = rw_mod<RW_NRX>(RPS * s + (RW_) + a);                 \
-            _Pragma("unroll") for (int kb = 0; kb < TKB; ++kb) vx[kb][a] = lane_b + (XBASE - 64 + kb * XPLANE + xi * ROWB + (PART_)); \
+            _Pragma("unroll") for (int kb = 0; kb < TKB; ++kb) vx[kb][a] = lane_x + (XBASE - 64 + kb * XPLANE + xi * ROWB + (PART_)); \
         }                                                                                                                  \
         _Pragma("unroll") for (int nb = 0; nb < TNB; ++nb)                                                                 \
             vd[nb] = lane_b + (DBASE + nb * DPLANE + ((RPS * s + (RW_)) & (RW_NRD - 1)) * ROWB + (PART_));                 \
-        float av[2][TNB], bv[2][TKB][9];                                                                                   \
+         \
+        const int vx3 = STEM ? (j < 8 ? vx[0][0] + 128 : vx[0][1] + 64) : 0;                                               \
+        (void)vx3;                                                                                                         \
+        float av[2][TNB], bv[2][TKB][NTAP];                                                                                \
         constexpr int NS_ = (STEPS + (F_) - 1) / (F_);                                                                     \
         DAM_RW_LOAD(0, 0);                                                                                                 \
         _Pragma("unroll") for (int t = 0; t < NS_; ++t) {                                                                  \
@@ -562,8 +575,8 @@
             if (t + 1 < NS_) DAM_RW_LOAD((F_) * (t + 1), (t + 1) & 1);                                                     \
             _Pragma("unroll") for (int nb = 0; nb < TNB; ++nb)                                                             \
                 _Pragma("unroll") for (int kb = 0; kb < TKB; ++kb)                                                         \
-                    _Pragma("unroll") for (int tap = 0; tap < 9; ++tap) {                                                  \
-                        const int idx = (nb * TKB + kb) * 9 + tap;                                                         \
+                    _Pragma("unroll") for (int tap = 0; tap < NTAP; ++tap) {                                               \
+                        const int idx = (nb * TKB + kb) * NTAP + tap;                                                      \
                         acc[idx] = __builtin_amdgcn_mfma_f32_16x16x4f32(av[t & 1][nb], bv[t & 1][kb][tap], acc[idx], 0, 0, 0); \
                     }                                                                                                      \
             DAM_RW_SCHED();                                                                                                \
@@ -604,7 +617,7 @@
         }
         __syncthreads();
     }
-    float4* out = reinterpret_cast<float4*>(partial) + ((size_t)by * gridDim.x + bx) * NBLK * 64;
+    float4* out = reinterpret_cast<float4*>(partial) + ((size_t)by * gridDim.x + bx) * NBLK_OUT * 64;
 #ifdef DAM_WGR_STAMPS
     DAM_WSTAMP(8);
     if (lane == 0 && (wave == 0 || wave == 4)) {
@@ -612,13 +625,23 @@
         for (int i = 0; i < 32; ++i) sp[i] = stamp_v[i];
     }
 #else
-    for (int e = tid; e < NBLK * 64; e += (256 + 64 * NL)) out[e] = reinterpret_cast<const float4*>(red)[e];
+    for (int e = tid; e < NBLK_OUT * 64; e += (256 + 64 * NL)) {
+        if constexpr (STEM) {
+            const int blk = e >> 6, l = e & 63, a = blk / 3, b = blk - a * 3;
+            const int src = b < 2 ? a : (a < 2 ? 3 : 4);
+            const bool upper = b == 1 || (b == 2 && a == 1);
+            const float4 v = reinterpret_cast<const float4*>(red)[src * 64 + (l & 55) + (upper ? 8 : 0)];
+            out[e] = (l & 8) ? make_float4(0.f, 0.f, 0.f, 0.f) : v;
+        } else {
+            out[e] = reinterpret_cast<const float4*>(red)[e];
+        }
+    }
 #endif
 }
 
 #undef DAM_RW_ZERO
 
-template <int TNB, int TKB, int STEPS, int KP, int GPP, int HV = 1, int NL = 8>
+template <int TNB, int TKB, int STEPS, int KP, int GPP, int HV = 1, int NL = 8, bool STEM = false>
 int launch_wgrad_rows(int B, int H, int W, int C, const float* X, const float* dY, const float* in_scale, const float* in_shift,
                       int relu_in, float* partial, int64_t ws_floats, float* dw, int n_real, int k_real, void* queue,
                       hipStream_t st) {
@@ -651,8 +674,8 @@
     }
     const int nsplit = B * g.spi;
     if ((int64_t)nsplit * nx * NBLK * 256 > ws_floats) return DAM_ERR_WORKSPACE;
-    if (!raise_lds_limit<&wgrad_rows_kernel<TNB, TKB, STEPS, KP, GPP, HV, NL>>(160 * 1024)) return DAM_ERR_LAUNCH;
-    hipLaunchKernelGGL((wgrad_rows_kernel<TNB, TKB, STEPS, KP, GPP, HV, NL>), dim3(nx, nsplit), dim3((256 + 64 * NL)), lds, st, g, X, dY, in_scale,
+    if (!raise_lds_limit<&wgrad_rows_kernel<TNB, TKB, STEPS, KP, GPP, HV, NL, STEM>>(160 * 1024)) return DAM_ERR_LAUNCH;
+    hipLaunchKernelGGL((wgrad_rows_kernel<TNB, TKB, STEPS, KP, GPP, HV, NL, STEM>), dim3(nx, nsplit), dim3((256 + 64 * NL)), lds, st, g, X, dY, in_scale,
                        in_shift, relu_in, partial);
     DAM_CHECK_LAUNCH();
     return reduce_submit(queue, partial, dw, nsplit, nx, TNB, TKB, 3, 3, n_real, k_real, 3, 3, 1, g.tiles_k, st);
@@ -1230,7 +1253,7 @@
     if (kh == 3 && kw == 3 && stride == 1 && pad == 1 && dil == 1 && !in_nchw && Ho == H && Wo == W && C == n_chan) {
         int rc = DAM_ERR_UNSUPPORTED;
 #define DAM_WGR(...) launch_wgrad_rows<__VA_ARGS__>(B, H, W, C, x, dy, in_scale, in_shift, relu_in, workspace, workspace_floats, dw, n_out, k_real, reduce_queue, st)
-        if (C == 16) { rc = DAM_WGR(1, 1, 33, 1, 9); if (rc == DAM_ERR_UNSUPPORTED) rc = DAM_WGR(1, 1, 28, 1, 14, 2); }
+        if (C == 16) { rc = (c_real > 0 && c_real <= 8) ? DAM_WGR(1, 1, 33, 1, 9, 1, 8, true) : DAM_WGR(1, 1, 33, 1, 9); if (rc == DAM_ERR_UNSUPPORTED) rc = DAM_WGR(1, 1, 28, 1, 14, 2); }
         else if (W > 80) rc = DAM_WGR(2, 1, 14, 1, 7, 2);
         else if (W > 48) { rc = DAM_WGR(2, 1, 17, 2, 5); if (rc == DAM_ERR_UNSUPPORTED) rc = DAM_WGR(2, 1, 14, 2, 4); }
         else if (W > 20) rc = DAM_WGR(2, 1, 9, 2, 3);
diff --git a/deep-audio-mixer_amd/layers.py b/deep-audio-mixer_amd/layers.py
--- a/deep-audio-mixer_amd/layers.py
+++ b/deep-audio-mixer_amd/layers.py
@@ -13,6 +13,7 @@
     def __init__(self, cin, cout, k, stride=1, pad=0, dil=1, in_nchw=False):
         self.cin, self.cout, self.k, self.stride, self.pad, self.dil, self.in_nchw = cin, cout, k, stride, pad, dil, in_nchw
         self.wp = self.wpt = None
+        self.c_real = None
         self.nhwc16 = None
         if in_nchw and k == 3 and stride == 1 and pad == 1 and dil == 1 and cin <= 16:
             self.nhwc16 = _Nhwc16Spec(self)
@@ -23,7 +24,7 @@
 
     def fwd(self, x, w, bias=None):
         return ops.conv2d_fwd(x, self.packed(w), self.cout, self.k, self.k, self.stride, self.pad, self.dil,
-                              bias=bias, in_nchw=self.in_nchw)
+                              bias=bias, in_nchw=self.in_nchw, c_real=self.c_real)
 
     def fwd_conv(self, x, w, bn, training, bias=None, in_affine=None, fuse_stats=True, finalize=True):
         wp = self.packed(w)
@@ -32,12 +33,13 @@
             n16 = (self.cout + 15) // 16 * 16
             buf = ops.bn_partial_buffer(x.device, n16)
             c, parts, out4 = ops.conv2d_fwd(x, wp, self.cout, self.k, self.k, self.stride, self.pad, self.dil, bias=bias,
-                                            bn_partial=buf, bn=_bn_args(bn, training), finalize=finalize, **aff)
+                                            bn_partial=buf, bn=_bn_args(bn, training), finalize=finalize, c_real=self.c_real,
+                                            **aff)
             if not finalize:
                 return c, ((buf, parts) if parts > 0 else None)
             return c, ((out4[0], out4[1], out4[2], out4[3]) if parts > 0 else None)
         return ops.conv2d_fwd(x, wp, self.cout, self.k, self.k, self.stride, self.pad, self.dil, bias=bias,
-                              in_nchw=self.in_nchw, **aff), None
+                              in_nchw=self.in_nchw, c_real=self.c_real, **aff), None
 
     def fwd_bn(self, x, w, bn, training, bias=None, in_affine=None):
         c, stats = self.fwd_conv(x, w, bn, training, bias=bias, in_affine=in_affine)
@@ -69,6 +71,7 @@
     def __init__(self, parent):
         self.cin, self.cout, self.k, self.stride, self.pad, self.dil, self.in_nchw = 16, parent.cout, 3, 1, 1, 1, False
         self.parent, self.nhwc16, self.wpt = parent, None, None
+        self.c_real = parent.cin
 
     @property
     def wp(self):
diff --git a/deep-audio-mixer_amd/ops.py b/deep-audio-mixer_amd/ops.py
--- a/deep-audio-mixer_amd/ops.py
+++ b/deep-audio-mixer_amd/ops.py
@@ -51,11 +51,11 @@
 
 def _tapgrid(x, B, H, W, C, in_nchw, wp, k_chunks, n_out, bias, in_scale, in_shift, relu_in, y, OHt, OWt, Ho, Wo,
              out_stride, oo_h, oo_w, in_stride, nA, nB, off_h, step_h, off_w, step_w, wt_base, wt_sa, wt_sb,
-             res=None, res_mask=None, bn_partial=None, relu_out=False, batch=None, bn_bwd=None):
+             res=None, res_mask=None, bn_partial=None, relu_out=False, batch=None, bn_bwd=None, c_real=None):
     parts = ctypes.c_int(0)
     ws = _workspace(y.device, min(8 * y.numel(), 8 * 400 * 64 * 64))
     st = _lib.lib().dam_conv2d_tapgrid_f32(
-        _lib.ptr(x), B, H, W, C, 1 if in_nchw else 0, _lib.ptr(wp), k_chunks, n_out, _lib.ptr(bias),
+        _lib.ptr(x), B, H, W, C, 0 if c_real is None else int(c_real), 1 if in_nchw else 0, _lib.ptr(wp), k_chunks, n_out, _lib.ptr(bias),
         _lib.ptr(in_scale), _lib.ptr(in_shift), 1 if relu_in else 0, 1 if relu_out else 0, _lib.ptr(y), OHt, OWt, Ho, Wo,
         out_stride,
         oo_h, oo_w, in_stride, nA, nB, off_h, step_h, off_w, step_w, wt_base, wt_sa, wt_sb, _lib.ptr(res),
@@ -68,7 +68,8 @@
 
 
 def conv2d_fwd(x, wp, n_out, kh, kw, stride=1, pad=0, dil=1, bias=None, in_scale=None, in_shift=None,
-               relu_in=False, in_nchw=False, bn_partial=None, bn=None, res=None, relu_out=False, finalize=True, out=None):
+               relu_in=False, in_nchw=False, bn_partial=None, bn=None, res=None, relu_out=False, finalize=True, out=None,
+               c_real=None):
     _lib.require_cuda(x, wp)
     _f32c(x, 'x'), _f32c(bias, 'bias'), _f32c(in_scale, 'in_scale'), _f32c(in_shift, 'in_shift'), _f32c(res, 'res')
     if in_nchw:
@@ -89,7 +90,7 @@
         y = out
     parts = _tapgrid(x, B, H, W, C, in_nchw, wp, k_chunks, n16, bias, in_scale, in_shift, relu_in, y, Ho, Wo, Ho, Wo,
                      1, 0, 0, stride, kh, kw, -pad, dil, -pad, dil, 0, kw, 1, res=res, bn_partial=bn_partial,
-                     relu_out=relu_out)
+                     relu_out=relu_out, c_real=c_real)
     if bn is not None and bn_partial is not None:
         out4 = bn_finalize(bn_partial, parts, *bn) if parts > 0 and finalize else None
         return y, parts, out4
@@ -99,13 +100,13 @@
 
 
 CONV_FAMILIES = ('none', 'strip', 'pipe', 'pipe_ranges', 'tile', 'tile_batch', '1x1')
-ConvLaunch = collections.namedtuple('ConvLaunch', 'family MB NB NCH T33 LW EPI SO PU STATS KS ksplit ranges')
+ConvLaunch = collections.namedtuple('ConvLaunch', 'family MB NB NCH T33 LW EPI SO PU STATS KS ksplit ranges STEM')
 
 
 def conv_last_launch():
     v = (ctypes.c_int * 16)()
     _lib.check(_lib.lib().dam_conv_last_launch(v), 'dam_conv_last_launch')
-    return ConvLaunch(CONV_FAMILIES[v[0]], *v[1:13])
+    return ConvLaunch(CONV_FAMILIES[v[0]], *v[1:14])
 
 
 def _dgrad_axis(parity, pad, dil, k, stride):
diff --git a/include/dam_hip.h b/include/dam_hip.h
--- a/include/dam_hip.h
+++ b/include/dam_hip.h
@@ -20,7 +20,7 @@
 #define DAM_PCM_ROTATE 0x200
 struct dam_bn_bwd_sums;
 
-#define DAM_ABI_VERSION 26
+#define DAM_ABI_VERSION 27
 const char* dam_arch(void);
 int dam_abi_version(void);
 
@@ -70,7 +70,7 @@
 
 int dam_conv_pack_weights_multi_f32(const int64_t* desc_dev, int n_tensors, int64_t max_total, void* stream);
 
-int dam_conv2d_tapgrid_f32(const float* x, int B, int H, int W, int C, int in_nchw, const float* w_packed,
+int dam_conv2d_tapgrid_f32(const float* x, int B, int H, int W, int C, int c_real, int in_nchw, const float* w_packed,
                            int k_chunks, int n_out, const float* bias, const float* in_scale,
                            const float* in_shift, int relu_in, int relu_out, float* y, int OHt, int OWt, int Ho, int Wo,
                            int out_stride, int out_off_h, int out_off_w, int in_stride, int nA, int nB,
```

Result: no change. 2.040 million stem-spectrogram-frames/s, median of 6 (+0.5%).
